# nickirk/pymes

Hardware: AMD Instinct MI355X
Metric: ccsd_iteration_time (lower is better)
Workload: dtype f64

## Files before the change

include/pymes_amd.h:

```cpp
#ifndef PYMES_AMD_H
#define PYMES_AMD_H

#include <stdint.h>

#ifdef __cplusplus
extern "C" {
#endif

typedef struct pymes_ctx pymes_ctx;

const char* pymes_last_error(void);
const char* pymes_backend(void);
int pymes_ctx_create(pymes_ctx** out, int device, int no, int nv, uint64_t workspace_bytes );
int pymes_ctx_destroy(pymes_ctx* ctx);
int pymes_ctx_set_stream(pymes_ctx* ctx, void* hip_stream);
int pymes_ctx_sync(pymes_ctx* ctx);
int pymes_ctx_workspace(pymes_ctx* ctx, uint64_t* capacity_bytes, uint64_t* high_water_bytes);

int pymes_malloc(pymes_ctx* ctx, uint64_t bytes, void** dev_ptr);
int pymes_free(pymes_ctx* ctx, void* dev_ptr);
int pymes_live_allocations(int64_t* n);
int pymes_mem_info(pymes_ctx* ctx, uint64_t* free_bytes, uint64_t* total_bytes);
int pymes_dress_generation(pymes_ctx* ctx, uint64_t* n);

// ... 154 lines not shown
                      double* e_out_host);
int pymes_ccd_energy(pymes_ctx* ctx, const double* t2_dev, double* e_out_host);

int pymes_ueg_eval_2b(pymes_ctx* ctx, int n_p, int n_ele, int imax, int mode, double L, double k_cutoff, double gamma,
                      int lattice_cutoff, const int32_t* k_int_host, const int32_t* index_map_host, double* V_dev);

int pymes_ueg_eval_2b_corr(pymes_ctx* ctx, int n_p, int n_ele, int imax, int mode, double L, int lattice_cutoff,
                           int correlator, const double* params_host, const int32_t* k_int_host,
                           const int32_t* index_map_host, double* V_dev);
int pymes_ueg_eval_2b_tab(pymes_ctx* ctx, int n_p, int n_ele, int imax, int mode, double L, int lattice_cutoff,
                          const int32_t* k_int_host, const int32_t* index_map_host, const double* tab_scalar_host,
                          const double* tab_array_host, int64_t tab_len, double* V_dev);

int pymes_dots(pymes_ctx* ctx, int npairs, const double* const* x_dev, const double* const* y_dev, int64_t n,
               double* out_host);
int pymes_dots_var(pymes_ctx* ctx, int npairs, const double* const* x_dev, const double* const* y_dev,
                   const int64_t* n, double* out_host);
int pymes_lincomb(pymes_ctx* ctx, double* out_dev, int nx, const double* const* x_dev, const double* c_host,
                  int64_t n);
int pymes_gemm_group_begin(pymes_ctx* ctx);
int pymes_gemm_group_end(pymes_ctx* ctx, int64_t* launches, int64_t* products);
int pymes_gram(pymes_ctx* ctx, int m, int n, const double* const* x_dev, const double* const* y_dev, int64_t len,
               double* out_host);
int pymes_lincomb_multi(pymes_ctx* ctx, int m, int n, const double* const* x_dev, const double* c_host,
                        const double* beta_host, double* const* y_dev, int64_t len);
int pymes_diis_mix(pymes_ctx* ctx, double* state_host, int ntypes, int m, int was_full, const double* const* err_hist_dev,
                   const double* const* err_new_dev, const int64_t* sizes, const double* const* amp_hist_dev,
                   double* const* out_dev);
int pymes_diis_step(pymes_ctx* ctx, double* state_dev, int npairs, const double* const* x_dev, const double* const* y_dev,
                    const int64_t* n, int ntypes, int m, int was_full);
int pymes_diis_solve(double* state_host, const double* overlaps_host, int ntypes, int m, int was_full);
int pymes_lincomb_dev(pymes_ctx* ctx, double* out_dev, int nx, const double* const* x_dev, const double* coeff_dev,
                      int64_t n);
int pymes_cmul(pymes_ctx* ctx, const double* mr_dev, const double* mi_dev, const double* xr_dev, const double* xi_dev,
               double* yr_dev, double* yi_dev, int64_t n);

int pymes_hf_fock_matrix(pymes_ctx* ctx, const double* h_host, double* f_host);

int pymes_fcidump_header(const char* path, int* n_elec, int* n_orb);
int pymes_fcidump_read_host(const char* path, int is_tc, double* e_core, double* eps_host, double* h_host,
                            double* V_host);
int pymes_fcidump_load(pymes_ctx* ctx, const char* path, int is_tc, double* e_core, double* eps_host, double* h_host,
                       int64_t* n_two_electron_lines);

int pymes_packed_header(const char* path, int* kind, int* n_elec, int* n_orb, int* naux);
int pymes_packed_load(pymes_ctx* ctx, const char* path, double* e_core, double* eps_host, double* h_host);
int pymes_packed_write(pymes_ctx* ctx, const char* path, int n_elec, double e_core, const double* eps_host,
                       const double* h_host);
int pymes_packed_write_factors(const char* path, int n_elec, int n_orb, int naux, double e_core, const double* eps_host,
                               const double* h_host, const double* B_host);

typedef struct pymes_eom pymes_eom;
int pymes_eom_sigma_prepare(pymes_ctx* ctx, const double* f_host, const double* t2_dev, int dressed, pymes_eom** out);
int pymes_eom_sigma_flags(pymes_eom* h, int* flags);
int pymes_eom_sigma_apply(pymes_eom* h, int k, const double* const* u1_dev, const double* const* u2_dev, const int* sym,
                          double* const* s1_dev, double* const* s2_dev);
int pymes_eom_diagonals(pymes_ctx* ctx, const double* f_host, const double* t2_dev, int dressed, double* d1_dev, double* d2_dev);
int pymes_scratch_trim(pymes_ctx* ctx);
int pymes_eom_sigma_destroy(pymes_eom* h);

#define PYMES_IPEA_IP 0
#define PYMES_IPEA_EA 1
typedef struct pymes_ipea pymes_ipea;
int pymes_ipea_sigma_prepare(pymes_ctx* ctx, const double* f_host, const double* t2_dev, int dressed, int kind, pymes_ipea** out);
int pymes_ipea_sigma_flags(pymes_ipea* h, int* flags);
int pymes_ipea_sigma_apply(pymes_ipea* h, int k, const double* const* r1_dev, const double* const* r2_dev, double* const* s1_dev,
// ... 44 lines not shown
```

pymes_amd/_lib.py:

```python
import ctypes as C
import os

import numpy as np

_HERE = os.path.dirname(os.path.abspath(__file__))
DEFAULT_PATH = os.environ.get("PYMES_AMD_LIBRARY") or os.path.join(_HERE, "lib", "libpymes_amd.so")

c_double_p = C.POINTER(C.c_double)
c_i64_p = C.POINTER(C.c_int64)


class ShardBuffers(C.Structure):
    _fields_ = [(k, C.c_void_p) for k in ("ETd", "ETx", "L", "QK", "Tall", "W", "Xvv", "P", "R1", "S")]

c_pp = C.POINTER(C.c_void_p)

SIGNATURES = {
    "pymes_last_error": (C.c_char_p, []),
    "pymes_backend": (C.c_char_p, []),
    "pymes_ctx_create": (C.c_int, [c_pp, C.c_int, C.c_int, C.c_int, C.c_uint64]),
    "pymes_ctx_destroy": (C.c_int, [C.c_void_p]),
    "pymes_ctx_set_stream": (C.c_int, [C.c_void_p, C.c_void_p]),
    "pymes_ctx_sync": (C.c_int, [C.c_void_p]),
    "pymes_ctx_workspace": (C.c_int, [C.c_void_p, C.POINTER(C.c_uint64), C.POINTER(C.c_uint64)]),
# ... 125 lines not shown
    "pymes_ccsd_sharded_finish": (C.c_int, [C.c_void_p] * 6 + [C.POINTER(C.c_int)]),
    "pymes_ccsd_sharded_energy": (C.c_int, [C.c_void_p, C.c_int, C.c_void_p]),
    "pymes_ccsd_sharded_await": (C.c_int, [C.c_void_p, C.c_void_p, C.c_void_p]),
    "pymes_cshift_inv": (C.c_int, [C.c_void_p, C.c_void_p] + [C.c_double] * 5 + [C.c_void_p, C.c_void_p, C.c_int64]),
    "pymes_eom_sigma_prepare": (C.c_int, [C.c_void_p, C.c_void_p, C.c_void_p, C.c_int, C.c_void_p]),
    "pymes_eom_sigma_flags": (C.c_int, [C.c_void_p, C.c_void_p]),
    "pymes_eom_sigma_apply": (C.c_int, [C.c_void_p, C.c_int] + [C.c_void_p] * 5),
    "pymes_eom_diagonals": (C.c_int, [C.c_void_p, C.c_void_p, C.c_void_p, C.c_int, C.c_void_p, C.c_void_p]),
    "pymes_scratch_trim": (C.c_int, [C.c_void_p]),
    "pymes_eom_sigma_destroy": (C.c_int, [C.c_void_p]),
    "pymes_eom_sigma_apply_left": (C.c_int, [C.c_void_p, C.c_int] + [C.c_void_p] * 5),
    "pymes_lambda_step": (C.c_int, [C.c_void_p] * 5 + [C.c_double, C.c_double, C.c_int, C.c_int] + [C.c_void_p] * 5),
    "pymes_rdm1": (C.c_int, [C.c_void_p] * 5 + [C.c_double, C.c_void_p]),
    "pymes_ipea_sigma_prepare": (C.c_int, [C.c_void_p, C.c_void_p, C.c_void_p, C.c_int, C.c_int, C.c_void_p]),
    "pymes_ipea_sigma_flags": (C.c_int, [C.c_void_p, C.c_void_p]),
    "pymes_ipea_sigma_apply": (C.c_int, [C.c_void_p, C.c_int] + [C.c_void_p] * 4),
    "pymes_ipea_sigma_apply_left": (C.c_int, [C.c_void_p, C.c_int] + [C.c_void_p] * 4),
    "pymes_ipea_dyson": (C.c_int, [C.c_void_p] * 4 + [C.c_int] + [C.c_void_p] * 6),
    "pymes_ipea_sigma_diagonals": (C.c_int, [C.c_void_p, C.c_void_p, C.c_void_p]),
    "pymes_ipea_sigma_correction": (C.c_int, [C.c_void_p, C.c_int, C.c_void_p, C.c_void_p, C.c_void_p, C.c_void_p, C.c_double,
                                              C.c_void_p, C.c_int64, C.c_int64, C.c_void_p]),
    "pymes_ipea_sigma_destroy": (C.c_int, [C.c_void_p]),
    "pymes_tdm1": (C.c_int, [C.c_void_p] * 5 + [C.c_int] + [C.c_void_p] * 7),
    "pymes_eom_correction": (C.c_int, [C.c_void_p, C.c_int, C.c_void_p, C.c_void_p, C.c_void_p, C.c_void_p, C.c_double,
                                       C.c_void_p, C.c_int64, C.c_int64, C.c_void_p]),
    "pymes_diis_mix": (C.c_int, [C.c_void_p, C.c_void_p, C.c_int, C.c_int, C.c_int, c_pp, c_pp, c_i64_p, c_pp, c_pp]),
    "pymes_diis_solve": (C.c_int, [C.c_void_p, C.c_void_p, C.c_int, C.c_int, C.c_int]),
    "pymes_diis_step": (C.c_int, [C.c_void_p, C.c_void_p, C.c_int, c_pp, c_pp, c_i64_p, C.c_int, C.c_int, C.c_int]),
    "pymes_gemm_group_begin": (C.c_int, [C.c_void_p]),
    "pymes_gemm_group_end": (C.c_int, [C.c_void_p, c_i64_p, c_i64_p]),
    "pymes_gram": (C.c_int, [C.c_void_p, C.c_int, C.c_int, c_pp, c_pp, C.c_int64, c_double_p]),
    "pymes_lincomb_multi": (C.c_int, [C.c_void_p, C.c_int, C.c_int, c_pp, C.c_void_p, C.c_void_p, c_pp, C.c_int64]),
    "pymes_lincomb_dev": (C.c_int, [C.c_void_p, C.c_void_p, C.c_int, c_pp, C.c_void_p, C.c_int64]),
    "pymes_stats": (C.c_int, [C.c_void_p, C.c_int, c_i64_p, c_double_p, c_i64_p, c_double_p]),
    "pymes_prof_enable": (C.c_int, [C.c_void_p, C.c_int]),
    "pymes_prof_reset": (C.c_int, [C.c_void_p]),
    "pymes_prof_query": (C.c_int, [C.c_void_p, C.c_int, c_i64_p, c_i64_p, c_double_p, c_double_p]),
}

PYMES_DCD, PYMES_USE_DRESSED, PYMES_SKIP_LADDER, PYMES_SYM_LADDER, PYMES_SYM_RINGS = 1, 2, 4, 8, 16
PYMES_OWNER_TILES = 1 << 21
PYMES_REUSE_LAYOUTS = 32
PYMES_T1_ZERO = 1 << 20
PYMES_SLAB_RINGS_ONLY, PYMES_SLAB_LADDERS_ONLY = 64, 128
PYMES_DRESS_ABIJ_REDUCED = 1 << 16


class PymesError(RuntimeError):
    pass


class Library:

    BACKEND = "hip-gfx950"

    def __init__(self, path=None):
        path = path or DEFAULT_PATH
        if not os.path.exists(path):
            raise PymesError(
                f"{path} not found: build the HIP extension first (python -c 'import __graft_entry__ as g; "
                "g.build()' or make -C pymes_amd/csrc).  pymes_amd has no CPU fallback.")
        self.path = path
        self.dll = C.CDLL(path)
        for name, (res, args) in SIGNATURES.items():
            fn = getattr(self.dll, name)
            fn.restype, fn.argtypes = res, args
        self.backend = self.dll.pymes_backend().decode()
        if self.backend != self.BACKEND:
            raise PymesError(f"{path} reports backend '{self.backend}', expected '{self.BACKEND}'")

    def call(self, name, *args):
        rc = getattr(self.dll, name)(*args)
        if rc != 0:
            raise PymesError(f"{name}: {self.dll.pymes_last_error().decode()}")


# ... 22 lines not shown
```

pymes_amd/csrc/capi.cpp:

```cpp
#include <chrono>
#include <cstdio>
#include <cstring>
#include <exception>
#include <algorithm>
#include <mutex>
#include <set>
#include <string>
#include <vector>

#include "../../include/pymes_amd.h"
#include "diis_small.h"
#include "engine.h"
#include "eom.h"
#include "fcidump.h"
#include "packed.h"

using pymes::Engine;
using pymes::TView;

struct pymes_ctx {
    Engine* e;
};
struct pymes_eom {
    pymes::EomSigma* s;
// ... 338 lines not shown
}
int pymes_shard_rows_ptr(pymes_ctx* ctx, const double** vp, const double** vm, int64_t* row0, int64_t* row1, int64_t* ldp,
                         int64_t* ldm) {
    return guarded([&] {
        need(vp, "vp"); need(vm, "vm"); need(row0, "row0"); need(row1, "row1"); need(ldp, "ldp"); need(ldm, "ldm");
        E(ctx).shard_rows(vp, vm, row0, row1, ldp, ldm);
    });
}
int pymes_set_orbital_energies(pymes_ctx* ctx, const double* eo, const double* ev) {
    return guarded([&] {
        need(eo, "eps_o");
        need(ev, "eps_v");
        E(ctx).set_orbital_energies(eo, ev);
    });
}

int pymes_mp2(pymes_ctx* ctx, double shift, double* t2, double* e_out) {
    return guarded([&] {
        need(t2, "t2");
        need(e_out, "e_out");
        E(ctx).mp2(shift, t2, e_out);
    });
}
int pymes_ccsd_dress_fock(pymes_ctx* ctx, const double* f, const double* t1, double* fd) {
    return guarded([&] {
        need(f, "f"); need(t1, "t1"); need(fd, "fd");
        E(ctx).dress_fock(f, t1, fd);
    });
}
int pymes_ccsd_residuals(pymes_ctx* ctx, const double* f, const double* t1, const double* t2, uint32_t flags, double* r1,
                         double* r2) {
    return guarded([&] {
        need(f, "f"); need(t1, "t1"); need(t2, "t2"); need(r1, "r1"); need(r2, "r2");
        if (flags & ~(PYMES_DCD | PYMES_T1_ZERO)) throw pymes::Error("ccsd_residuals: flags are PYMES_DCD | PYMES_T1_ZERO");
        E(ctx).ccsd_residuals(f, t1, t2, (flags & PYMES_DCD) | ((flags & PYMES_T1_ZERO) ? Engine::kT1Zero : 0u), r1, r2);
    });
}
int pymes_ccsd_iterate(pymes_ctx* ctx, const double* f, double* t1, double* t2, uint32_t flags, double level_shift, double delta,
                       double* dt1, double* dt2, double* out6) {
    return guarded([&] {
        need(f, "f"); need(t1, "t1"); need(t2, "t2"); need(dt1, "dt1"); need(dt2, "dt2"); need(out6, "out");
        if (flags & ~(PYMES_DCD | PYMES_T1_ZERO)) throw pymes::Error("ccsd_iterate: flags are PYMES_DCD | PYMES_T1_ZERO");
        Engine& e = E(ctx);
        if (e.capturing()) throw pymes::Error("ccsd_iterate reads the energy back: not inside a launch graph");
        e.ccsd_iterate(f, t1, t2, (flags & PYMES_DCD) | ((flags & PYMES_T1_ZERO) ? Engine::kT1Zero : 0u), level_shift, delta, dt1,
                       dt2, out6);
    });
}
int pymes_ccsd_release(pymes_ctx* ctx) {
    return guarded([&] {
        Engine& e = E(ctx);
        if (e.capturing()) throw pymes::Error("ccsd_release while a launch graph is being recorded");
        e.release_residual_buffers();
    });
}
int pymes_ccsd_dress_V(pymes_ctx* ctx, const double* t1, uint32_t mask) {
    return guarded([&] {
        need(t1, "t1");
        E(ctx).dress_V(t1, mask);
    });
}
int pymes_ccsd_dress_V_slab(pymes_ctx* ctx, const double* t1, uint32_t mask, int p_begin, int p_end, int q_begin,
                            int q_end) {
    return guarded([&] {
        need(t1, "t1");
        const int64_t cut[4] = {p_begin, p_end, q_begin, q_end};
        E(ctx).dress_V(t1, mask, cut);
    });
// ... 187 lines not shown
}
int pymes_ccsd_dress_abcd_rows(pymes_ctx* ctx, const double* t1, int a0, int a1, int lower_only) {
    return guarded([&] {
        need(t1, "t1");
        E(ctx).dress_abcd_rows(t1, a0, a1, lower_only != 0);
    });
}
int pymes_cc_update(pymes_ctx* ctx, double* t, double* dt, const double* r, double shift, double delta, int rank) {
    return guarded([&] {
        need(t, "t"); need(dt, "dt"); need(r, "r");
        E(ctx).cc_update(t, dt, r, shift, delta, rank);
    });
}
int pymes_cc_update_to(pymes_ctx* ctx, double* t_out, double* dt, const double* t_in, const double* r, double shift,
                       double delta, int rank) {
    return guarded([&] {
        need(t_out, "t_out"); need(dt, "dt"); need(t_in, "t_in"); need(r, "r");
        E(ctx).cc_update_to(t_out, dt, t_in, r, shift, delta, rank);
    });
}
int pymes_energy_norms(pymes_ctx* ctx, const double* f, const double* t1, const double* t2, const double* dt2,
                       double* out) {
    return guarded([&] {
        need(t2, "t2"); need(out, "out");
        if ((f == nullptr) != (t1 == nullptr)) throw pymes::Error("f and t1 must be given together");
        E(ctx).energy_norms(f, t1, t2, dt2, out);
    });
}
int pymes_energy_norms_start(pymes_ctx* ctx, const double* f, const double* t1, const double* t2, const double* dt2, int* slot) {
    return guarded([&] {
        need(t2, "t2"); need(slot, "slot");
        if ((f == nullptr) != (t1 == nullptr)) throw pymes::Error("f and t1 must be given together");
        *slot = E(ctx).energy_norms_start(f, t1, t2, dt2);
    });
}
int pymes_energy_norms_wait(pymes_ctx* ctx, int slot, double* out) {
    return guarded([&] {
        need(out, "out");
        Eq(ctx).energy_norms_wait(slot, out);
    });
}
int pymes_readback_start(pymes_ctx* ctx, const double* dev_ptr, int n, int* slot) {
    return guarded([&] {
        need(dev_ptr, "dev_ptr"); need(slot, "slot");
        *slot = dev::readback_start(dev_ptr, n, E(ctx).stream);
    });
}
int pymes_readback_wait(pymes_ctx* ctx, int slot, double* out, int n) {
    return guarded([&] {
        need(out, "out");
        Eq(ctx);
        dev::readback_wait(slot, out, n);
    });
}
int pymes_energy_norms_pairs(pymes_ctx* ctx, const double* f, const double* t1, const double* tc, const double* dtc,
                             int rank, int world, double* out) {
    return guarded([&] {
        need(tc, "tc"); need(out, "out");
        if ((f == nullptr) != (t1 == nullptr)) throw pymes::Error("f and t1 must be given together");
        E(ctx).energy_norms_pairs(f, t1, tc, dtc, rank, world, out);
    });
}
int pymes_set_collectives(pymes_ctx* ctx, const pymes_collectives* table) {
    return guarded([&] {
        if (!table) {
            E(ctx).set_collectives(nullptr);
// ... 137 lines not shown
        need(params, "params");
        if (mode == 0) throw pymes::Error("ueg: mode 0 (Coulomb) has no correlator");
        if (correlator < 1 || correlator > 6) throw pymes::Error("ueg: correlator must be 1..6 (0 = trunc: pymes_ueg_eval_2b)");
        ueg_eval(ctx, n_p, n_ele, imax, mode, L, 0.0, 1.0, lattice_cutoff, k_int, index_map, nullptr, nullptr, 0, V, correlator, params);
    });
}
int pymes_ueg_eval_2b_tab(pymes_ctx* ctx, int n_p, int n_ele, int imax, int mode, double L, int lattice_cutoff,
                          const int32_t* k_int, const int32_t* index_map, const double* tab_scalar, const double* tab_array,
                          int64_t tab_len, double* V) {
    return guarded([&] {
        need(tab_scalar, "tab_scalar"); need(tab_array, "tab_array");
        if (mode == 0) throw pymes::Error("ueg: mode 0 (Coulomb) has no correlator");
        ueg_eval(ctx, n_p, n_ele, imax, mode, L, 0.0, 1.0, lattice_cutoff, k_int, index_map, tab_scalar, tab_array, tab_len, V);
    });
}

int pymes_dots(pymes_ctx* ctx, int npairs, const double* const* x, const double* const* y, int64_t n,
               double* out) {
    return guarded([&] {
        need(x, "x"); need(y, "y"); need(out, "out");
        if (npairs < 0 || npairs > 16) throw pymes::Error("dots: 0..16 pairs");
        int64_t len[16];
        for (int i = 0; i < npairs; ++i) len[i] = n;
        dev::dots(npairs, x, y, len, out, E(ctx).stream);
    });
}
int pymes_dots_var(pymes_ctx* ctx, int npairs, const double* const* x, const double* const* y, const int64_t* n,
                   double* out) {
    return guarded([&] {
        need(x, "x"); need(y, "y"); need(n, "n"); need(out, "out");
        dev::dots(npairs, x, y, n, out, E(ctx).stream);
    });
}
int pymes_lincomb(pymes_ctx* ctx, double* out, int nx, const double* const* x, const double* c, int64_t n) {
    return guarded([&] {
        need(out, "out"); need(x, "x"); need(c, "c");
        dev::lincomb(out, nx, x, c, n, E(ctx).stream);
    });
}

int pymes_gemm_group_begin(pymes_ctx* ctx) {
    return guarded([&] { dev::gemm_group_begin(Eq(ctx).stream); });
}
int pymes_gemm_group_end(pymes_ctx* ctx, int64_t* launches, int64_t* products) {
    return guarded([&] {
        Eq(ctx);
        dev::gemm_group_end();
        long l = 0, p = 0;
        dev::gemm_group_stats(&l, &p);
        if (launches) *launches = l;
        if (products) *products = p;
    });
}
int pymes_gram(pymes_ctx* ctx, int m, int n, const double* const* x, const double* const* y, int64_t len, double* out) {
    return guarded([&] {
        need(x, "x"); need(y, "y"); need(out, "out");
        if (m < 0 || n < 0 || len < 0) throw pymes::Error("gram: negative size");
        for (int i = 0; i < m; ++i) need(x[i], "x[i]");
        for (int j = 0; j < n; ++j) need(y[j], "y[j]");
        dev::gram(m, n, x, y, len, out, E(ctx).stream);
    });
}
int pymes_lincomb_multi(pymes_ctx* ctx, int m, int n, const double* const* x, const double* c, const double* beta,
                        double* const* y, int64_t len) {
    return guarded([&] {
        need(y, "y");
        if (m < 0 || n < 0 || len < 0) throw pymes::Error("lincomb_multi: negative size");
        if (m > 0) { need(x, "x"); need(c, "c"); }
        for (int i = 0; i < m; ++i) need(x[i], "x[i]");
        for (int j = 0; j < n; ++j) need(y[j], "y[j]");
        dev::lincomb_multi(m, n, x, c, beta, y, len, E(ctx).stream);
    });
}

int pymes_diis_step(pymes_ctx* ctx, double* state, int npairs, const double* const* x, const double* const* y, const int64_t* n,
                    int ntypes, int m, int was_full) {
    return guarded([&] {
        need(state, "state"); need(x, "x"); need(y, "y"); need(n, "n");
        dev::diis_step(state, npairs, x, y, n, ntypes, m, was_full, E(ctx).stream);
    });
}
int pymes_diis_solve(double* state_host, const double* overlaps_host, int ntypes, int m, int was_full) {
    return guarded([&] {
        need(state_host, "state"); need(overlaps_host, "overlaps");
        if (ntypes < 1 || m < 1 || m > 8) throw pymes::Error("diis_solve: need ntypes >= 1, 1 <= m <= 8");
        diis_small::step(state_host, overlaps_host, ntypes, m, was_full);
    });
}
int pymes_diis_mix(pymes_ctx* ctx, double* state_host, int ntypes, int m, int was_full, const double* const* err_hist,
                   const double* const* err_new, const int64_t* sizes, const double* const* amp_hist, double* const* out) {
    return guarded([&] {
        need(state_host, "state"); need(err_hist, "err_hist"); need(err_new, "err_new"); need(sizes, "sizes");
        need(amp_hist, "amp_hist"); need(out, "out");
        if (ntypes < 1 || m < 1 || m > 8 || ntypes * m > 16) throw pymes::Error("diis_mix: need ntypes * m <= 16, m <= 8");
        Engine& e = E(ctx);
        const double* x[16];
        const double* y[16];
        int64_t n[16];
        for (int t = 0; t < ntypes; ++t)
            for (int i = 0; i < m; ++i) {
                x[t * m + i] = err_hist[t * m + i];
                y[t * m + i] = err_new[t];
                n[t * m + i] = sizes[t];
            }
        double ov[16];
        dev::dots(ntypes * m, x, y, n, ov, e.stream);
        diis_small::step(state_host, ov, ntypes, m, was_full);
        if (state_host[91] == 2.0)
            throw pymes::Error("DIIS: the subspace matrix is singular or not finite (numpy.linalg.LinAlgError in pymes/mixer/diis.py:85-95)");
        for (int t = 0; t < ntypes; ++t) dev::lincomb(out[t], m, amp_hist + t * m, state_host + 82, sizes[t], e.stream);
    });
}
int pymes_lincomb_dev(pymes_ctx* ctx, double* out, int nx, const double* const* x, const double* coeff_dev, int64_t n) {
    return guarded([&] {
        need(out, "out"); need(x, "x"); need(coeff_dev, "coeff");
        dev::lincomb_dev(out, nx, x, coeff_dev, n, E(ctx).stream);
    });
}
int pymes_cmul(pymes_ctx* ctx, const double* mr, const double* mi, const double* xr, const double* xi, double* yr, double* yi,
               int64_t n) {
    return guarded([&] {
        need(mr, "mr"); need(mi, "mi"); need(xr, "xr"); need(xi, "xi"); need(yr, "yr"); need(yi, "yi");
        dev::cmul(mr, mi, xr, xi, yr, yi, n, E(ctx).stream);
    });
}

int pymes_cshift_inv(pymes_ctx* ctx, const double* d, double zr, double zi, double hr, double hi, double shift, double* mr,
                     double* mi, int64_t n) {
    return guarded([&] {
        need(d, "d"); need(mr, "mr"); need(mi, "mi");
        dev::cshift_inv(d, zr, zi, hr, hi, shift, mr, mi, n, E(ctx).stream);
    });
}

int pymes_eom_sigma_prepare(pymes_ctx* ctx, const double* f_host, const double* t2, int dressed, pymes_eom** out) {
    return guarded([&] {
        need(out, "out");
        *out = nullptr;
        need(f_host, "f_host"); need(t2, "t2");
        Engine& e = E(ctx);
        e.refuse_if_sharded("EOM sigma");
        if (e.capturing()) throw pymes::Error("eom_sigma_prepare while a launch graph is being recorded");
        pymes::EomSigma* s = new pymes::EomSigma(e, f_host, t2, dressed != 0);
// ... 383 lines not shown
```

pymes_amd/csrc/cc.cpp:

```cpp
#include <algorithm>
#include <cstdio>
#include <cstring>
#include <cstdlib>
#include <vector>

#include "../../include/pymes_amd.h"
#include "engine.h"

#include <cmath>

namespace pymes {
static_assert(Engine::kT1Zero == PYMES_T1_ZERO && Engine::kOwnerTiles == PYMES_OWNER_TILES,
              "the engine's flag bits are the public ones");

namespace {
inline int64_t lpitch(int64_t n) { return (n + 15) & ~int64_t(15); }
inline TView packed_rows(double* p, int64_t rows, int64_t cols) { return slice(make_view(p, {rows, lpitch(cols)}), 1, 0, cols); }
constexpr int P_klij = 0, P_ijka = 1, P_ijak = 2, P_ijab = 3, P_iajk = 4, P_iajb = 5, P_iabj = 6, P_iabc = 7,
              P_aibc = 11, P_abij = 12, P_abic = 13, P_abci = 14, P_abcd = 15;
}

double* Engine::get_static(const std::string& key) {
    auto it = static_.find(key);
    if (it != static_.end()) return it->second;
// ... 130 lines not shown
            ArenaScope s2(arena);
            TView Z = ov2(), Q = ov2();
            contract(1.0, Td, "dkai", Vx, "cldk", 0.0, Z, "aicl");
            permute(-1.0, T, "cblj", 0.0, Q, "clbj");
            permute(1.0, T, "bclj", 1.0, Q, "clbj");
            contract(1.0, Z, "aicl", Q, "clbj", 1.0, Exd, "aibj");
        }
        Rx = ov2();
        TView X1 = ov2();
        contract(1.0, Tx, "ajdk", Vx, "cldk", 0.0, X1, "ajcl");
        contract(1.0, X1, "ajcl", Tx, "clbi", 0.0, Rx, "ajbi");
    }

    permute(1.0, Rd, "aibj", 1.0, R, "abij");
    if (quad) permute(1.0, Rx, "ajbi", 1.0, R, "abij");
    permute(1.0, Exd, "aibj", 1.0, R, "abij");
    permute(1.0, Exd, "bjai", 1.0, R, "abij");
    permute(1.0, Exx, "ajbi", 1.0, R, "abij");
    permute(1.0, Exx, "biaj", 1.0, R, "abij");
    permute(1.0, Exn, "abij", 1.0, R, "abij");
    permute(1.0, Exn, "baji", 1.0, R, "abij");
}

void Engine::ensure_xs() {
    if (!xs_oo_) xs_oo_ = static_cast<double*>(dev::dmalloc(sizeof(double) * no * no));
    if (!xs_vv_) xs_vv_ = static_cast<double*>(dev::dmalloc(sizeof(double) * nv * nv));
}

bool Engine::ring_fold_enabled() {
    if (const char* e = getenv("PYMES_RING_FOLD")) return atoi(e) != 0;
    return true;
}

void Engine::pair_layouts_of(const double* t2, bool want_td) {
    const int64_t o = no, v = nv, ov = o * v;
    for (int i = want_td ? 0 : 1; i < 3; ++i)
        if (!lay_[i]) {
            if (capturing_) throw Error("pair_layouts_of: the pair layouts must exist before a launch graph is recorded (run one eager pass first)");
            lay_[i] = static_cast<double*>(dev::dmalloc(sizeof(double) * ov * ov));
        }
    lay_t2_ = nullptr;
    if (dev::fused_pair_kernels_ok(no)) {
        dev::t2_layouts(t2, want_td ? lay_[0] : nullptr, lay_[1], lay_[2], no, nv, stream);
        stats.permute_calls++;
        stats.permute_bytes += 8.0 * (want_td ? 5.0 : 4.0) * double(ov * ov);
    } else {
        TView T = make_view(const_cast<double*>(t2), {v, v, o, o});
        TView t4 = make_view(lay_[0], {v, o, v, o});
        if (want_td) permute(1.0, T, "abij", 0.0, t4, "aibj");
        t4.p = lay_[1];
        permute(1.0, T, "abij", 0.0, t4, "ajbi");
        t4.p = lay_[2];
        permute(2.0, T, "abij", 0.0, t4, "aibj");
        permute(-1.0, T, "baij", 1.0, t4, "aibj");
    }
    lay_t2_ = t2;
}

void Engine::residual_slab(const double* f, const double* t2, double* ETd_p, double* ETx_p, double* L, int rank,
                           int world, unsigned flags, const double* t1, double* QK, const double* P) {
    const bool dcd = flags & PYMES_DCD, dressed = flags & PYMES_USE_DRESSED,
               skip_ladder = flags & (PYMES_SKIP_LADDER | PYMES_SLAB_RINGS_ONLY), skip_rings = flags & PYMES_SLAB_LADDERS_ONLY;
    const bool quad = !dcd;
    const int64_t o = no, v = nv, nn = n, ov = o * v;
    if (world < 1 || rank < 0 || rank >= world) throw Error("residual_slab: bad rank/world");
    if (L && !skip_ladder) check_shard_rank("residual_slab", rank, world);
    const double w = quad ? 1.0 : 0.5;
    TView F = make_view(const_cast<double*>(f), {nn, nn});
    auto chunk = [&](int64_t rows, int64_t& lo, int64_t& hi) {
        const int64_t c = (rows + world - 1) / world;
        lo = std::min<int64_t>(rank * c, rows);
        hi = std::min<int64_t>(lo + c, rows);
    };
    if (L && !skip_ladder) {
        int64_t r0, r1;
        chunk(v * (v + 1) / 2, r0, r1);
        if (t1) {
            if (!QK) throw Error("residual_slab: QK buffer missing");
            int64_t q0, q1;
            chunk(o * v, q0, q1);
            ladder_t1(t1, t2, L, r0, r1, QK, q0, q1, dcd, P ? P + o * o : nullptr);
        } else {
            ladder_sym(t2, L, r0, r1, dressed, quad ? 1 : 2);
        }
    }
    if (skip_rings) return;
    ring_fold_.clear();
    int64_t c0, c1;
    chunk(ov, c0, c1);
    const int64_t nc = c1 - c0;
    if (nc <= 0) return;
    TView Viajb = block(P_iajb, dressed), Viabj = block(P_iabj, dressed);

    ArenaScope scope(arena);
    auto pairm = [&](double* p) { return make_view(p, {ov, ov}); };
    auto slab = [&]() { return make_view(arena.alloc(ov * nc), {ov, nc}); };
    const bool traces = !P && nc == ov;
    const bool fold = traces && ring_fold_enabled();
    pair_layouts_of(t2, !fold);
    TView Td = pairm(lay_[0]), Tx = pairm(lay_[1]), Ttd = pairm(lay_[2]);
    TView ETd = slice(pairm(ETd_p), 0, c0, c1), ETx = slice(pairm(ETx_p), 0, c0, c1);
    auto cols = [&](const TView& m) { return slice(m, 1, c0, c1); };
    const int64_t b0 = c0 / o, b1 = (c1 + o - 1) / o;
    auto load_cols = [&](double alpha, const TView& blk, const char* spec, const TView& dst) {
        TView src = slice(blk, 1, b0, b1);
        if (b0 * o == c0 && b1 * o == c1) {
            permute(alpha, src, spec, 0.0, make_view(dst.p, {v, o, b1 - b0, o}), "ckbj");
        } else {
            ArenaScope s2(arena);
            TView tmp = make_view(arena.alloc(ov * (b1 - b0) * o), {ov, (b1 - b0) * o});
            permute(alpha, src, spec, 0.0, make_view(tmp.p, {v, o, b1 - b0, o}), "ckbj");
            copy(slice(tmp, 1, c0 - b0 * o, c1 - b0 * o), dst);
        }
    };
    const bool row_form = nc != ov;
    if (row_form) {
        auto slabT = [&]() { return make_view(arena.alloc(nc * ov), {nc, ov}); };
        TView MT = slabT(), N1T = slabT();
        auto load_rows = [&](double alpha, const TView& blk, const char* spec, const TView& dst) {
            TView src = slice(blk, 1, b0, b1);
            if (b0 * o == c0 && b1 * o == c1) {
                permute(alpha, src, spec, 0.0, make_view(dst.p, {b1 - b0, o, v, o}), "bjck");
            } else {
                ArenaScope s2(arena);
                TView tmp = make_view(arena.alloc((b1 - b0) * o * ov), {(b1 - b0) * o, ov});
                permute(alpha, src, spec, 0.0, make_view(tmp.p, {b1 - b0, o, v, o}), "bjck");
                copy(slice(tmp, 0, c0 - b0 * o, c1 - b0 * o), dst);
            }
        };
        load_rows(2.0, Viabj, "kbcj", MT);
        load_rows(-1.0, Viajb, "kbjc", N1T);
        axpby(1.0, N1T, 1.0, MT);
// ... 1120 lines not shown
        contract(-1.0, t, "ak", S2, "ki", 1.0, R, "ai");
    }
    contract(-1.0, Tq, "ajbk", slice(block(P_ijka), 0, j0, j1), "jkib", 1.0, R, "ai");
    if (!have_vv) {
        TView S4 = make_view(arena.alloc(v * v), {v, v});
        contract(1.0, Tq, "ajbk", slice(block(P_ijab), 0, j0, j1), "jkcb", 0.0, S4, "ac");
        contract(-1.0, S4, "ac", t, "ci", 1.0, R, "ai");
    }
}

void Engine::cc_update(double* t, double* dt, const double* r, double shift, double delta, int rank) {
    if (rank != 2 && rank != 4) throw Error("cc_update: rank must be 2 (T1) or 4 (T2)");
    need_eps("cc_update");
    dev::cc_update(t, dt, r, eps_o, eps_v, shift, delta, no, nv, rank, stream);
}

void Engine::ccsd_residuals(const double* f, const double* t1, const double* t2, unsigned flags, double* r1, double* r2) {
    refuse_if_sharded("ccsd_residuals (single rank)");
    const int64_t o = no, v = nv, ov = o * v, npp = v * (v + 1) / 2;
    if (!res_ETd_) {
        if (capturing_) throw Error("ccsd_residuals: the staging buffers must exist before a launch graph is recorded (run one eager pass first)");
        double* got[5] = {nullptr, nullptr, nullptr, nullptr, nullptr};
        const int64_t want[5] = {(o + v) * (o + v), ov * ov, ov * ov, npp * o * o, ov * o * o};
        try {
            for (int i = 0; i < 5; ++i) got[i] = scratch_get(want[i]);
        } catch (...) {
            for (double* p : got)
                if (p) scratch_put(p);
            throw;
        }
        res_fd_ = got[0]; res_ETd_ = got[1]; res_ETx_ = got[2]; res_L_ = got[3]; res_QK_ = got[4];
    }
    const unsigned dcd = flags & PYMES_DCD;
    const unsigned sym = PYMES_SYM_LADDER | PYMES_SYM_RINGS;
    if (flags & PYMES_T1_ZERO) {
        residual_slab(f, t2, res_ETd_, res_ETx_, res_L_, 0, 1, dcd | sym);
        singles_residual_partial(f, t1, t2, r1, 0, 1, true);
        residual_finish(f, t2, res_ETd_, res_ETx_, res_L_, r2, dcd | sym | PYMES_REUSE_LAYOUTS);
        return;
    }
    dress_fock(f, t1, res_fd_);
    dress_V(t1, (1u << pattern_of_name("klij")) | (1u << pattern_of_name("iajb")) | (1u << pattern_of_name("iabj")));
    residual_slab(res_fd_, t2, res_ETd_, res_ETx_, res_L_, 0, 1, dcd | sym | PYMES_USE_DRESSED, t1, res_QK_);
    singles_residual_partial(res_fd_, t1, t2, r1, 0, 1, true);
    residual_finish(res_fd_, t2, res_ETd_, res_ETx_, res_L_, r2, dcd | sym | PYMES_USE_DRESSED | PYMES_REUSE_LAYOUTS, t1, res_QK_);
}

void Engine::ccsd_iterate(const double* f, double* t1, double* t2, unsigned flags, double shift, double delta, double* dt1,
                          double* dt2, double out[6]) {
    refuse_if_sharded("ccsd_iterate (single rank)");
    const int64_t o = no, v = nv;
    if (!res_r1_) {
        if (capturing_) throw Error("ccsd_iterate: the staging buffers must exist before a launch graph is recorded");
        double* r1 = scratch_get(v * o);
        try {
            res_r2_ = scratch_get(v * v * o * o);
        } catch (...) {
            scratch_put(r1);
            throw;
        }
        res_r1_ = r1;
    }
    ccsd_residuals(f, t1, t2, flags, res_r1_, res_r2_);
    cc_update_to(t1, dt1, t1, res_r1_, shift, delta, 2);
    cc_update_to(t2, dt2, t2, res_r2_, shift, delta, 4);
    energy_norms(f, t1, t2, dt2, out);
}

void Engine::set_collectives(const Collectives* c) {
    if (t2_in_flight_) {
        t2_in_flight_ = false;
        dev::phase_sync();
        if (coll_.wait(coll_.user, t2_ticket_, stream) != 0) throw Error("collective hook: wait failed");
    }
    if (!c) {
        coll_ = Collectives();
        coll_set_ = false;
        return;
    }
    if (!c->allreduce_start || !c->allgather_start || !c->wait) throw Error("set_collectives: allreduce_start, allgather_start and wait are required");
    if (c->world < 1 || c->rank < 0 || c->rank >= c->world) throw Error("set_collectives: need 0 <= rank < world");
    coll_ = *c;
    coll_set_ = true;
}

namespace {
struct Hooks {
    const Engine::Collectives& c;
    void* stream;
    int64_t allreduce(double* buf, int64_t n) const {
        dev::gemm_group_sync();
        dev::phase_sync();
        int64_t t = 0;
        if (c.allreduce_start(c.user, buf, n, stream, &t) != 0) throw Error("collective hook: allreduce_start failed");
        return t;
    }
    int64_t allgather(double* buf, int64_t chunk) const {
        dev::gemm_group_sync();
        dev::phase_sync();
// ... 206 lines not shown
                                stream);
    h.wait(h.allreduce(b.S, 6));
    const int slot = dev::readback_start(b.S, 6, stream);
    t2_ticket_ = h.allgather(b.Tall, c * 2 * o2);
    t2_in_flight_ = true;
    h.mark("energy + norms (pairs)");
    return slot;
}

void Engine::ccsd_sharded_energy(int slot, double out[6]) {
    double r[6];
    dev::readback_wait(slot, r, 6);
    out[0] = 2.0 * r[0];
    out[1] = 2.0 * r[1];
    out[2] = -1.0 * r[2];
    out[3] = r[3];
    out[4] = r[4];
    out[5] = r[5];
}

void Engine::release_residual_buffers() {
    if (!graphs_.empty()) {
        release_wanted_ = true;
        return;
    }
    release_wanted_ = false;
    for (double** p : {&res_fd_, &res_ETd_, &res_ETx_, &res_L_, &res_QK_, &res_r1_, &res_r2_}) {
        if (*p) scratch_put(*p);
        *p = nullptr;
    }
}

void Engine::cc_update_to(double* t_out, double* dt, const double* t_in, const double* r, double shift, double delta,
                          int rank) {
    if (rank != 2 && rank != 4) throw Error("cc_update: rank must be 2 (T1) or 4 (T2)");
    need_eps("cc_update");
    dev::cc_update_to(t_out, dt, t_in, r, eps_o, eps_v, shift, delta, no, nv, rank, stream);
}

int Engine::energy_norms_start(const double* f, const double* t1, const double* t2, const double* dt2) {
    return dev::energy_norms_start(f, t1, t2, get_static("Edir"), get_static("Eex"), dt2, no, nv, stream);
}
void Engine::energy_norms_wait(int slot, double out[6]) {
    double r[6];
    dev::readback_wait(slot, r, 6);
    out[0] = 2.0 * r[0];
    out[1] = 2.0 * r[1];
    out[2] = -1.0 * r[2];
    out[3] = r[3];
    out[4] = r[4];
    out[5] = r[5];
}

void Engine::energy_norms(const double* f, const double* t1, const double* t2, const double* dt2, double out[6]) {
    double r[6];
    dev::energy_norms(f, t1, t2, get_static("Edir"), get_static("Eex"), dt2, no, nv, r, stream);
    out[0] = 2.0 * r[0];
    out[1] = 2.0 * r[1];
    out[2] = -1.0 * r[2];
    out[3] = r[3];
    out[4] = r[4];
    out[5] = r[5];
}

void Engine::energy_norms_pairs(const double* f, const double* t1, const double* tc, const double* dtc, int rank, int world,
                                double out[6]) {
    int64_t r0, r1;
    pair_chunk(rank, world, r0, r1);
    double r[6];
    dev::energy_norms_pairs(f, t1, tc, get_static("Edir"), get_static("Eex"), dtc, no, nv, r0, r1, rank == 0, r, stream);
    out[0] = 2.0 * r[0];
    out[1] = 2.0 * r[1];
    out[2] = -1.0 * r[2];
    out[3] = r[3];
    out[4] = r[4];
    out[5] = r[5];
}

void Engine::ccsd_energy(const double* f, const double* t1, const double* t2, double out[3]) {
    double r[6];
    energy_norms(f, t1, t2, nullptr, r);
    out[0] = r[0];
    out[1] = r[1];
    out[2] = r[2];
}

void Engine::ccd_energy(const double* t2, double out[2]) {
// ... 426 lines not shown
```

pymes_amd/csrc/device_api.h:

```cpp
#pragma once
#include <cstddef>
#include <cstdint>

namespace dev {

typedef void* stream_t;

const char* backend_name();
void  set_device(int ordinal);
void* dmalloc(size_t bytes);
void* try_dmalloc(size_t bytes);
void  dfree(void* p);
void  memcpy_h2d(void* d, const void* h, size_t bytes, stream_t s);
void  memcpy_d2h(void* h, const void* d, size_t bytes, stream_t s);
void  memcpy_d2d(void* d, const void* s_, size_t bytes, stream_t s);
void  memset_zero(void* d, size_t bytes, stream_t s);
void  stream_sync(stream_t s);
size_t mem_free_bytes();
size_t mem_total_bytes();
stream_t stream_create();
void  stream_destroy(stream_t s);
int64_t live_allocations();
typedef void* event_t;
event_t event_create();
// ... 48 lines not shown
void phase_stats(long* tasks, long* launches, long* levels, long* flushes);

struct Permute {
    int rank;
    int64_t dim[6];
    int64_t s_in[6], s_out[6];
    double alpha, beta;
    const double* in; double* out;
};
void permute(const Permute& p, stream_t s);

void mp2_amplitudes(double* t, const double* w, const double* eo, const double* ev, double shift,
                    int no, int nv, stream_t s);
void cc_update(double* t, double* dt, const double* r, const double* eo, const double* ev, double shift,
               double delta, int no, int nv, int rank, stream_t s);
void dots(int npairs, const double* const* x, const double* const* y, const int64_t* n, double* out_host,
          stream_t s);
void energy_norms(const double* f, const double* t1, const double* t2, const double* Edir, const double* Eex,
                  const double* dt2, int no, int nv, double out_host[6], stream_t s);
int energy_norms_start(const double* f, const double* t1, const double* t2, const double* Edir, const double* Eex,
                       const double* dt2, int no, int nv, stream_t s);
int readback_start(const double* dev_ptr, int n, stream_t s);
void readback_wait(int slot, double* out_host, int n);
void energy_norms_pairs(const double* f, const double* t1, const double* tc, const double* Edir, const double* Eex,
                        const double* dtc, int no, int nv, int64_t r0, int64_t r1, bool with_t1, double out_host[6],
                        stream_t s);
void energy_norms_pairs_dev(const double* f, const double* t1, const double* tc, const double* Edir, const double* Eex,
                            const double* dtc, int no, int nv, int64_t r0, int64_t r1, bool with_t1, double* out_dev,
                            stream_t s);
void exchange_asymmetry(const double* A, const double* B, const int64_t d[4], double out_host[2], stream_t s);
void cc_update_to(double* t_out, double* dt, const double* t_in, const double* r, const double* eo, const double* ev,
                  double shift, double delta, int no, int nv, int rank, stream_t s);
void lincomb(double* out, int nx, const double* const* x, const double* c, int64_t n, stream_t s);
void gram(int m, int n, const double* const* x, const double* const* y, int64_t len, double* out_host, stream_t s);
void lincomb_multi(int m, int n, const double* const* x, const double* c, const double* beta, double* const* y, int64_t len,
                   stream_t s);
void diis_step(double* state, int npairs, const double* const* x, const double* const* y, const int64_t* n, int ntypes, int m,
               int was_full, stream_t s);
void lincomb_dev(double* out, int nx, const double* const* x, const double* coeff_dev, int64_t n, stream_t s);
void cmul(const double* mr, const double* mi, const double* xr, const double* xi, double* yr, double* yi, int64_t n, stream_t s);
void exchange_split(const double* u, double* us, double* w, double* dg, int no, int nv, stream_t s);
void sgn_ij_add(double* D, const double* R, int no, int nv, stream_t s);
void cshift_inv(const double* d, double zr, double zi, double hr, double hi, double shift, double* mr, double* mi, int64_t n,
                stream_t s);
int64_t eom_diag_ws_doubles(int no, int nv);
void eom_diagonals(const double* V, const double* T, const double* dai, const double* iaai, const double* iaia, const double* ijij,
                   const double* abab, double* d1, double* d2, int no, int nv, double* ws, stream_t s);
void tau_build(double* tau, const double* t2, const double* t1, int no, int nv, stream_t s);

void ladder_pack_V(const double* V, double* Vp, double* Vm, int nr, int nc, int64_t rp0, int64_t rp1, stream_t s,
                   int64_t ldvp = 0, int64_t ldvm = 0);
void ladder_pack_V_factors(const double* B, double* Vp, double* Vm, int naux, int n, int no, int64_t rp0, int64_t rp1,
                           stream_t s, int64_t ldvp, int64_t ldvm);
int64_t triples_partial_doubles(int nv, int64_t nt);
void triples_energy(const double* W, int64_t nt, int64_t t0, const double* Vijab, const double* t1, const double* eps,
                    double* partial, double* out, int no, int nv, stream_t s);
int64_t fno_density_partial_doubles(int noa, int nv);
void fno_density(const double* Vijab, const double* eps_o, const double* eps_v, int no, int nf, int nv, double* partial,
                 double* D, double* e, stream_t s);
bool ladder_dress_ok(int no, int nv);
int64_t ladder_dress_ws_doubles(int no, int nv);
void ladder_dress(const double* V, const double* Pk, const double* t1, double* W, int no, int nv, int64_t ld, int64_t row0,
                  int64_t row1, double sgn, double* ws, stream_t s);
enum { PACK_ROW_HALF = 1, PACK_AM_PROWS = 2, PACK_COL_HALF = 4, PACK_AM_PCOLS = 8 };
void ladder_pack_T(const double* X, const double* t1, double* Sp, double* Am, int nc, int nr, int flags, int64_t ldp,
                   int64_t ldm, stream_t s, int64_t rp0 = 0, int64_t rp1 = -1);
// ... 88 lines not shown
```

pymes_amd/csrc/engine.cpp:

```cpp
#include "engine.h"

#include <algorithm>
#include <cstdio>
#include <cstdlib>
#include <cstring>
#include <tuple>

namespace pymes {

TView make_view(double* p, int rank, const int64_t* dims, const int64_t* strides) {
    if (rank < 0 || rank > 6) throw Error("tensor rank must be 0..6");
    TView t;
    t.p = p;
    t.rank = rank;
    int64_t s = 1;
    for (int i = rank - 1; i >= 0; --i) {
        t.dim[i] = dims[i];
        t.st[i] = strides ? strides[i] : s;
        s *= dims[i];
    }
    return t;
}
TView make_view(double* p, std::initializer_list<int64_t> dims) {
    int64_t d[6];
// ... 731 lines not shown
                                     double*, double*, stream_t) {
    throw std::runtime_error("ipea_pack: not available in this backend");
}
__attribute__((weak)) void ipea_assemble(int, const double*, const double*, const double*, const double*, int, int, int,
                                         double* const*, double* const*, stream_t) {
    throw std::runtime_error("ipea_assemble: not available in this backend");
}
__attribute__((weak)) void ipea_unpack(int, const double*, const double*, const double*, const double*, const double*, int, int, int,
                                       double* const*, double* const*, stream_t) {
    throw std::runtime_error("ipea_unpack: not available in this backend");
}
__attribute__((weak)) void ipea_dyson_assemble(const DysonParts&, int, int, int, int, stream_t) {
    throw std::runtime_error("ipea_dyson_assemble: not available in this backend");
}
__attribute__((weak)) void ipea_diagonals(const double*, const double*, int, int, int, double*, double*, stream_t) {
    throw std::runtime_error("ipea_diagonals: not available in this backend");
}
__attribute__((weak)) int64_t ipea_correction_ws_doubles(int, int64_t) { return 1; }
__attribute__((weak)) void ipea_correction(int, const double* const*, const double* const*, const double*, const double*, double,
                                           double* const*, int64_t, int64_t, int64_t, double*, double*, stream_t) {
    throw std::runtime_error("ipea_correction: not available in this backend");
}
__attribute__((weak)) int64_t lambda_assemble_ws_doubles(int) { return 1; }
__attribute__((weak)) void lambda_assemble(const LambdaParts&, int, int, stream_t) {
    throw std::runtime_error("lambda_assemble: not available in this backend");
}
__attribute__((weak)) void rdm1_assemble(const double*, const double*, const double*, const double*, const double*, int, int,
                                         double, double*, stream_t) {
    throw std::runtime_error("rdm1_assemble: not available in this backend");
}
__attribute__((weak)) void tdm1_assemble(const Tdm1Parts&, int, int, int, stream_t) {
    throw std::runtime_error("tdm1_assemble: not available in this backend");
}
}
```

pymes_amd/csrc/engine.h:

```cpp
#pragma once
#include <cstdint>
#include <map>
#include <set>
#include <stdexcept>
#include <string>
#include <vector>

#include "device_api.h"

namespace pymes {

struct TView {
    double* p = nullptr;
    int rank = 0;
    int64_t dim[6] = {1, 1, 1, 1, 1, 1};
    int64_t st[6] = {0, 0, 0, 0, 0, 0};
    int64_t size() const {
        int64_t n = 1;
        for (int i = 0; i < rank; ++i) n *= dim[i];
        return n;
    }
};

TView make_view(double* p, std::initializer_list<int64_t> dims);
// ... 106 lines not shown
    void singles_residual(const double* fd, const double* t1, const double* t2, double* r1);
    void singles_residual_partial(const double* fd, const double* t1, const double* t2, double* r1, int rank, int world,
                                  bool reuse_layouts = false);
    void doubles_residual(const double* f, const double* t2, double* r2, unsigned flags);
    void ladder(const double* t2, double* r2, int a0, int a1, bool dressed, double beta);
    void ladder_sym(const double* t2, double* L, int64_t row0, int64_t row1, bool dressed, int hole = 0);
    void ladder_sym_multi(const double* const* xs, int k, double* L_all, bool dressed);
    void ladder_sym_adjoint(const double* x, double* LS, double* LA, bool dressed);
    void ladder_sym_adjoint_multi(const double* const* xs, int k, double* LS, double* LA, bool dressed);
    int64_t ladder_adjoint_pitch(bool symmetric_half) const {
        const int64_t o = no, opp = o * (o + 1) / 2, opm = o * (o - 1) / 2;
        return ((symmetric_half ? opp : opm) + 2) & ~int64_t(1);
    }
    void hole_ladder_packed_multi(const double* const* xs, const double* const* Is, const double* const* ys, int k, double* L_all);
    void hole_ladder_packed(const double* x, const double* I, double* L, int64_t row0, int64_t row1,
                            const double* y = nullptr);
    void ladder_sym_unpack(const double* L, double* r2, double beta);
    void residual_slab(const double* f, const double* t2, double* ETd, double* ETx, double* L, int rank, int world,
                       unsigned flags, const double* t1 = nullptr, double* QK = nullptr, const double* P = nullptr);
    int64_t slab_prepare_ws_doubles() const;
    void slab_prepare(const double* t2, double* P, int rank, int world, unsigned flags);
    void residual_finish(const double* f, const double* t2, const double* ETd, const double* ETx, const double* L,
                         double* r2, unsigned flags, const double* t1 = nullptr, const double* QK = nullptr);
    void residual_finish_pairs(const double* f, const double* t2, const double* ETd, const double* ETx, const double* L,
                               double* Rc, unsigned flags, const double* t1, const double* QK, int rank, int world,
                               const double* Xvv_in = nullptr);
    void pair_chunk(int rank, int world, int64_t& r0, int64_t& r1) const;
    void amplitude_side_abij(const double* t1, const double* QK, const TView& N, int64_t a0, int64_t a1, int64_t b1,
                             bool with_partner, double beta = 1.0);
    void ladder_t1(const double* t1, const double* t2, double* L, int64_t row0, int64_t row1, double* QK, int64_t q0,
                   int64_t q1, bool dcd, const double* J = nullptr);
    void dress_abcd_rows(const double* t1, int a0, int a1, bool lower_only);
    static constexpr unsigned kT1Zero = 1u << 20;
    void ccsd_residuals(const double* f, const double* t1, const double* t2, unsigned flags, double* r1, double* r2);
    void ccsd_iterate(const double* f, double* t1, double* t2, unsigned flags, double shift, double delta, double* dt1,
                      double* dt2, double out[6]);
    void release_residual_buffers();
    void cc_update(double* t, double* dt, const double* r, double shift, double delta, int rank);
    void cc_update_to(double* t_out, double* dt, const double* t_in, const double* r, double shift, double delta, int rank);
    void ccsd_energy(const double* f, const double* t1, const double* t2, double out[3]);
    void ccd_energy(const double* t2, double out[2]);
    void energy_norms(const double* f, const double* t1, const double* t2, const double* dt2, double out[6]);
    int energy_norms_start(const double* f, const double* t1, const double* t2, const double* dt2);
    void energy_norms_wait(int slot, double out[6]);
    void energy_norms_pairs(const double* f, const double* t1, const double* tc, const double* dtc, int rank, int world,
                            double out[6]);
    struct Collectives {
        void* user = nullptr;
        int rank = 0, world = 1;
        int (*allreduce_start)(void* user, double* buf, int64_t n, void* stream, int64_t* ticket) = nullptr;
        int (*allgather_start)(void* user, double* buf, int64_t chunk, void* stream, int64_t* ticket) = nullptr;
        int (*wait)(void* user, int64_t ticket, void* stream) = nullptr;
        void (*mark)(void* user, const char* phase) = nullptr;
    };
    struct ShardBuffers {
        double *ETd, *ETx, *L, *QK, *Tall, *W, *Xvv, *P, *R1, *S;
    };
    void set_collectives(const Collectives* c);
    bool has_collectives() const { return coll_set_; }
    typedef int (*alltoallv_fn)(void* user, const double* send, const int64_t* send_counts, double* recv,
                                const int64_t* recv_counts, void* stream, int64_t* ticket);
    void set_alltoallv(alltoallv_fn fn) { alltoallv_ = fn; }
    void set_owner_tile_buffers(double* send, double* recv) { xs_ = send; xr_ = recv; }
    void owner_tile_sizes(int rank, int world, int64_t* send_doubles, int64_t* recv_doubles) const;
    static constexpr unsigned kOwnerTiles = 1u << 21;
    void ccsd_sharded_residuals(const double* f, double* fd, const double* t1, double* t2, const ShardBuffers& b,
                                unsigned flags, double* rc);
    void ccd_sharded_residuals(const double* f, double* t2, const ShardBuffers& b, unsigned flags, double* rc);
    int ccsd_sharded_finish(const double* f, const double* t1, const double* tc, const double* dtc, const ShardBuffers& b);
    void ccsd_sharded_energy(int slot, double out[6]);
    void ccsd_sharded_await(double* t2, const ShardBuffers& b);
    static int64_t triples_count(int no);
    double ccsd_t(const double* eps_host, const double* t1, const double* t2, int64_t t_begin, int64_t t_end, double* per_triple);
    void check_hermitian(const char* who, const char* why);
    double fno_density(const double* Vijab, int n_frozen, double* D_host);
    void derive_from(Engine& src, int n_frozen, const double* C_host, int nv_dst);
    void invalidate_static();

    double* eps_o = nullptr;
    double* eps_v = nullptr;
    bool eps_set = false;
    void need_eps(const char* who) const;
    double* splitk_ws() const { return splitk_ws_; }
    int64_t splitk_ws_doubles() const { return splitk_doubles_; }

  private:
    double* lay_[3] = {nullptr, nullptr, nullptr};
    const double* lay_t2_ = nullptr;
    void pair_layouts_of(const double* t2, bool want_td);
    struct FoldTag {
        const double* t2 = nullptr;
        const double* etd = nullptr;
        bool is(const double* t, const double* e) const { return t2 && t2 == t && etd == e; }
        void set(const double* t, const double* e) { t2 = t; etd = e; }
        void clear() { t2 = etd = nullptr; }
    } ring_fold_;
    static bool ring_fold_enabled();
    struct SumTag {
        const double* t2 = nullptr;
        int rank = 0, world = 0;
        bool is(const double* p, int r, int w) const { return t2 && t2 == p && rank == r && world == w; }
        void set(const double* p, int r, int w) { t2 = p; rank = r; world = w; }
        void clear() { t2 = nullptr; }
    };
    double ring_xd_ = 0.0;
    double* xs_oo_ = nullptr;
    double* xs_vv_ = nullptr;
    SumTag xs_oo_tag_, xs_vv_tag_;
    void ensure_xs();
    dev::stream_t own_stream_ = nullptr;
    std::set<void*> user_allocs_;
    Collectives coll_;
    alltoallv_fn alltoallv_ = nullptr;
    double *xs_ = nullptr, *xr_ = nullptr;
    struct Rect { int64_t r0, r1, c0, c1; };
    std::vector<Rect> owner_tile_rects(int from, int to, int world) const;
    int64_t owner_tiles_start(const ShardBuffers& b);
    void owner_tiles_finish(const ShardBuffers& b);
    bool coll_set_ = false, t2_in_flight_ = false;
    int64_t t2_ticket_ = 0;
    double *res_fd_ = nullptr, *res_ETd_ = nullptr, *res_ETx_ = nullptr, *res_L_ = nullptr, *res_QK_ = nullptr, *res_r1_ = nullptr,
           *res_r2_ = nullptr;
// ... 47 lines not shown
```

pymes_amd/csrc/kernels.hip:

```cpp
#include <hip/hip_runtime.h>
#include <type_traits>

#include <algorithm>
#include <atomic>
#include <chrono>
#include <cmath>
#include <cstdio>
#include <cstdlib>
#include <cstring>
#include <mutex>
#include <stdexcept>
#include <string>
#include <vector>

#include "device_api.h"
#include "diis_small.h"

#define HIP_CHECK(expr)                                                                   \
    do {                                                                                  \
        hipError_t err__ = (expr);                                                        \
        if (err__ != hipSuccess)                                                          \
            throw std::runtime_error(std::string("HIP error: ") + hipGetErrorString(err__) + \
                                     " at " __FILE__ ":" + std::to_string(__LINE__));     \
    } while (0)
// ... 2108 lines not shown
    const int p = no + 1;
    const long o2 = (long)no * no, ov = (long)no * nv, opp = (long)no * (no + 1) / 2;
    const long ab = ((long)a * nv + b) * o2, ba = ((long)b * nv + a) * o2;
    const long tab = (long)a * no * ov + (long)b * no, tba = (long)b * no * ov + (long)a * no;
    for (int e = threadIdx.x; e < o2; e += blockDim.x) {
        const int i = e / no, j = e - i * no;
        double v = N[ab + e] + D[tab + (long)i * ov + j] + X[tba + (long)i * ov + j];
        if (xd != 0.0) v += xd * X[tab + (long)i * ov + j];
        S[i * p + j] = v;
    }
    __syncthreads();
    for (int e = threadIdx.x; e < o2; e += blockDim.x) {
        const int j = e / no, i = e - j * no;
        double v = N[ba + e] + D[tba + (long)j * ov + i] + X[tab + (long)j * ov + i];
        if (xd != 0.0) v += xd * X[tba + (long)j * ov + i];
        S[i * p + j] += v;
    }
    __syncthreads();
    const double* __restrict__ row = L ? L + ((long)a * (a + 1) / 2 + b) * o2 : nullptr;
    for (int e = threadIdx.x; e < o2; e += blockDim.x) {
        const int i = e / no, j = e - i * no;
        const int ih = max(i, j), il = min(i, j);
        double ls = 0.0, la = 0.0;
        if (row) {
            ls = row[(long)ih * (ih + 1) / 2 + il];
            if (a != b && i != j) la = row[opp + (long)ih * (ih - 1) / 2 + il];
        }
        const double sgn = i > j ? 1.0 : -1.0;
        R[ab + e] = (V ? V[ab + e] : 0.0) + ls + sgn * la + S[i * p + j];
        if (a != b) R[ba + e] = (V ? V[ba + e] : 0.0) + ls - sgn * la + S[j * p + i];
    }
}
__global__ void __launch_bounds__(256) residual_assemble_kernel(const AssembleK k) { residual_assemble_body(k, blockIdx.x); }

__global__ void __launch_bounds__(256) energy_norms_pairs_kernel(const double* __restrict__ f, const double* __restrict__ t1,
                                                                 const double* __restrict__ tc, const double* __restrict__ Edir,
                                                                 const double* __restrict__ Eex, const double* __restrict__ dtc,
                                                                 int no, int nv, long r0, long npairs, int with_t1,
                                                                 double* __restrict__ partial) {
    __shared__ double sh[4];
    double s1 = 0.0, s2 = 0.0, s3 = 0.0, s4 = 0.0, s0 = 0.0, s5 = 0.0;
    const long o2 = (long)no * no;
    for (long tile = blockIdx.x; tile < 2 * npairs; tile += gridDim.x) {
        int a, b;
        unrank_pair(r0 + (tile >> 1), a, b);
        if (tile & 1) {
            if (a == b) continue;
            const int x = a; a = b; b = x;
        }
        const double* __restrict__ x = tc + tile * o2;
        const double* __restrict__ d = dtc ? dtc + tile * o2 : nullptr;
        const double* __restrict__ ed = Edir + ((long)a * nv + b) * o2;
        const double* __restrict__ ex = Eex + ((long)a * nv + b) * o2;
        for (int e = threadIdx.x; e < o2; e += blockDim.x) {
            const double v = x[e];
            double tau = v;
            if (t1) {
                const int i = e / no, j = e - i * no;
                tau += t1[a * no + i] * t1[b * no + j];
            }
            s1 += tau * ed[e];
            s2 += tau * ex[e];
            s3 += v * v;
            if (d) s4 += d[e] * d[e];
        }
    }
// ... 2033 lines not shown
        for (int i = 0; i < r; ++i) { k.dim[i] = m[i].n; k.s_in[i] = m[i].si; k.s_out[i] = m[i].so; }
        for (int i = r; i < 6; ++i) { k.dim[i] = 1; k.s_in[i] = 0; k.s_out[i] = 0; }
        if (phase) { record(PK_PERM_DIRECT, grid_for(total, 256, 256 * 32), 0, PermTaskK{k, total, 0, 0}); return; }
        launch_kernel(permute_direct_kernel, dim3(grid_for(total, 256, 256 * 32)), dim3(256), 0, st, k, total);
    }
}

void mp2_amplitudes(double* t, const double* w, const double* eo, const double* ev, double shift, int no, int nv,
                    stream_t s) {
    const long total = (long)nv * nv * no * no;
    if (!total) return;
    launch_kernel(mp2_amplitudes_kernel, dim3(grid_for(total)), dim3(256), 0, (hipStream_t)s, t, w, eo, ev,
                       shift, no, nv, total);
}

void cc_update_to(double* t_out, double* dt, const double* t_in, const double* r, const double* eo, const double* ev,
                  double shift, double delta, int no, int nv, int rank, stream_t s) {
    const long total = rank == 4 ? (long)nv * nv * no * no : (long)nv * no;
    if (!total) return;
    const CcUpdateK k{t_out, dt, t_in, r, eo, ev, shift, delta, no, nv, rank, total};
    const double cost = 32.0 * (double)total / 4.0e6;
    if (phase_open((hipStream_t)s) && phase_small(cost)) {
        PhaseRec& t = phase_push(PK_CC_UPDATE, 0, grid_for(total), 0, cost, k);
        phase_reads(t, {prange(t_in, total), prange(r, total), prange(eo, no), prange(ev, nv)});
        phase_writes(t, {prange(t_out, total), prange(dt, total)});
        return;
    }
    launch_kernel(cc_update_kernel, dim3(grid_for(total)), dim3(256), 0, (hipStream_t)s, k);
}
void cc_update(double* t, double* dt, const double* r, const double* eo, const double* ev, double shift,
               double delta, int no, int nv, int rank, stream_t s) {
    cc_update_to(t, dt, t, r, eo, ev, shift, delta, no, nv, rank, s);
}

static int launch_dots_stage1(int npairs, const double* const* x, const double* const* y, const int64_t* n, double* ws,
                              hipStream_t st) {
    DotPtrs p;
    long nmax = 0;
    bool vec = true;
    for (int i = 0; i < npairs; ++i) {
        p.x[i] = x[i]; p.y[i] = y[i]; p.n[i] = (long)n[i];
        nmax = std::max(nmax, p.n[i]);
        vec = vec && ((reinterpret_cast<uintptr_t>(x[i]) | reinterpret_cast<uintptr_t>(y[i])) & 15) == 0;
    }
    for (int i = npairs; i < 16; ++i) { p.x[i] = nullptr; p.y[i] = nullptr; p.n[i] = 0; }
    const long per = vec ? 512 : 256;
    const int nb = (int)std::max<long>(1, std::min<long>(kDotBlocks, (nmax + per - 1) / per));
    const DotsK k{p, ws, nb, npairs};
    double bytes = 0.0;
    for (int i = 0; i < npairs; ++i) bytes += 16.0 * (double)p.n[i];
    if (phase_open(st) && phase_small(bytes / 4.0e6)) {
        PhaseRec& t = phase_push(PK_DOTS1, vec ? 1 : 0, (long)nb * npairs, 0, bytes / 4.0e6, k);
        uintptr_t lo = ~(uintptr_t)0, hi = 0;
        for (int i = 0; i < npairs; ++i)
            for (const double* q : {p.x[i], p.y[i]}) {
                lo = std::min(lo, reinterpret_cast<uintptr_t>(q));
                hi = std::max(hi, reinterpret_cast<uintptr_t>(q) + 8 * (uintptr_t)p.n[i]);
            }
        phase_reads(t, {PhaseRange{lo, hi}});
        phase_writes(t, {prange(ws, 16L * kDotBlocks)});
        return nb;
    }
    if (vec) launch_kernel(dots_stage1_kernel<2>, dim3(nb * npairs), dim3(256), 0, st, k);
    else launch_kernel(dots_stage1_kernel<1>, dim3(nb * npairs), dim3(256), 0, st, k);
    return nb;
}
static void launch_dots_stage2(int npairs, double* ws, int nb, double* out_dev, hipStream_t st) {
    if (phase_open(st)) {
        PhaseRec& t = phase_push(PK_DOTS2, 0, npairs, 0, 1.0, Dots2K{ws, out_dev, nb});
        phase_reads(t, {prange(ws, 16L * kDotBlocks)});
        phase_writes(t, {prange(out_dev, npairs)});
        return;
    }
    launch_kernel(dots_stage2_kernel, dim3(npairs), dim3(256), 0, st, ws, nb, out_dev);
}

static void launch_dots_final(DotsFinalK k, double* ws, hipStream_t st) {
    {
        const int dv = current_device();
        std::lock_guard<std::mutex> lock(g_arrivals_mu);
        k.arrivals = g_arrivals[dv] + 32 * (g_arrivals_next[dv]++ % kArrivalSlots);
        k.pad_ = 0;
    }
    if (phase_open(st)) {
        PhaseRec& t = phase_push(PK_DOTS_FINAL, 0, k.npairs, 0, 1.0, k);
        phase_reads(t, {prange(ws, 16L * kDotBlocks)});
        return;
    }
    launch_kernel(dots_final_kernel, dim3(k.npairs), dim3(256), 0, st, k);
}

void dots(int npairs, const double* const* x, const double* const* y, const int64_t* n, double* out_host, stream_t s) {
    if (npairs <= 0) return;
    if (npairs > 16) throw std::runtime_error("dots: at most 16 pairs per call");
    hipStream_t st = (hipStream_t)s;
    const int dv = current_device();
    ensure_dot_ws(dv);
    const int nb = launch_dots_stage1(npairs, x, y, n, g_dot_ws[dv], st);
    void* hd = nullptr;
    HIP_CHECK(hipHostGetDevicePointer(&hd, g_dot_host[dv], 0));
    const long seq = ++g_dot_seq[dv];
    launch_dots_final(DotsFinalK{g_dot_ws[dv], static_cast<double*>(hd), reinterpret_cast<long*>(static_cast<double*>(hd) + 16), nullptr, 0u, seq, nb,
                                 npairs},
                      g_dot_ws[dv], st);
    phase_flush();
    if (!poll_flag(reinterpret_cast<const long*>(g_dot_host[dv] + 16), seq, st)) throw std::runtime_error("dots: the device never delivered the result");
    for (int i = 0; i < npairs; ++i) out_host[i] = g_dot_host[dv][i];
}

void diis_step(double* state, int npairs, const double* const* x, const double* const* y, const int64_t* n, int ntypes, int m,
               int was_full, stream_t s) {
    if (npairs != ntypes * m || npairs < 1 || npairs > 16 || m + 1 > diis_small::kMaxOrder)
        throw std::runtime_error("diis_step: bad sizes");
    hipStream_t st = (hipStream_t)s;
    const int dv = current_device();
    ensure_dot_ws(dv);
    const int nb = launch_dots_stage1(npairs, x, y, n, g_dot_ws[dv], st);
    double* out_dev = g_dot_ws[dv] + 16 * kDotBlocks;
    launch_dots_stage2(npairs, g_dot_ws[dv], nb, out_dev, st);
    launch_kernel(diis_step_kernel, dim3(1), dim3(64), 0, st, state, out_dev, ntypes, m, was_full);
}

void lincomb_dev(double* out, int nx, const double* const* x, const double* coeff_dev, int64_t n, stream_t s) {
    if (nx < 0 || nx > 8) throw std::runtime_error("lincomb_dev: at most 8 terms");
    if (n <= 0) return;
    LinPtrsDev p;
    for (int i = 0; i < 8; ++i) p.x[i] = i < nx ? x[i] : nullptr;
    launch_kernel(lincomb_dev_kernel, dim3(grid_for(n)), dim3(256), 0, (hipStream_t)s, out, p, coeff_dev, nx, (long)n);
}

int energy_norms_start(const double* f, const double* t1, const double* t2, const double* Edir, const double* Eex,
                       const double* dt2, int no, int nv, stream_t s) {
    gemm_group_flush();
    hipStream_t st = (hipStream_t)s;
    const int dv = current_device();
    ensure_dot_ws(dv);
    const long total = (long)nv * nv * no * no;
    const int nb = (int)std::max<long>(1, std::min<long>(kDotBlocks, (total + 255) / 256));
    const bool vec = (no % 2 == 0) && !((reinterpret_cast<uintptr_t>(t2) | reinterpret_cast<uintptr_t>(Edir) |
                                          reinterpret_cast<uintptr_t>(Eex) | reinterpret_cast<uintptr_t>(dt2)) & 15);
    const EnergyK k{f, t1, t2, Edir, Eex, dt2, g_dot_ws[dv], total, no, nv};
    const double cost = (dt2 ? 32.0 : 24.0) * (double)total / 4.0e6;
    if (phase_open(st) && phase_small(cost)) {
        PhaseRec& t = phase_push(PK_ENERGY, vec ? 1 : 0, nb, 0, cost, k);
        const long n = no + nv;
        phase_reads(t, {prange(t2, total), prange(Edir, total), prange(Eex, total), prange(dt2, dt2 ? total : 0),
                        prange(t1, t1 ? (long)no * nv : 0), prange(f, (t1 && f) ? n * n : 0)});
        phase_writes(t, {prange(g_dot_ws[dv], 16L * kDotBlocks)});
    } else {
        if (vec) launch_kernel(energy_norms_kernel<2>, dim3(nb), dim3(256), 0, st, k);
        else launch_kernel(energy_norms_kernel<1>, dim3(nb), dim3(256), 0, st, k);
    }
    double* out_pin = nullptr;
    long* flag = nullptr;
    long seq = 0;
    const int ticket = readback_reserve_flagged(dv, &out_pin, &flag, &seq);
    launch_dots_final(DotsFinalK{g_dot_ws[dv], out_pin, flag, nullptr, 0u, seq, nb, 6}, g_dot_ws[dv], st);
    phase_flush();
    return ticket;
}
void energy_norms(const double* f, const double* t1, const double* t2, const double* Edir, const double* Eex,
                  const double* dt2, int no, int nv, double out_host[6], stream_t s) {
    readback_wait_impl(energy_norms_start(f, t1, t2, Edir, Eex, dt2, no, nv, s), out_host, 6);
}
int readback_start(const double* dev_ptr, int n, stream_t s) {
    flush_deferred();
    return readback_start_impl(dev_ptr, n, (hipStream_t)s);
}
void readback_wait(int slot, double* out_host, int n) { readback_wait_impl(slot, out_host, n); }

void exchange_asymmetry(const double* A, const double* B, const int64_t d[4], double out_host[2], stream_t s) {
    hipStream_t st = (hipStream_t)s;
    const int dv = current_device();
    ensure_dot_ws(dv);
    const long total = (long)d[0] * d[1] * d[2] * d[3];
    out_host[0] = out_host[1] = 0.0;
    if (!total) return;
    unsigned long long* out_dev = reinterpret_cast<unsigned long long*>(g_dot_ws[dv] + 16 * kDotBlocks);
    HIP_CHECK(set_async(out_dev, 0, 2 * sizeof(unsigned long long), st));
    const long tr = (d[2] + 63) / 64, ts = (d[3] + 63) / 64, ntiles = d[0] * d[1] * tr * ts;
    const int self = (A == B && d[0] == d[1]) ? 1 : 0;
    const unsigned grid = (unsigned)std::min<long>(ntiles, 256L * 8);
    const bool vec = even(d[2]) && even(d[3]) && aligned16(A) && aligned16(B);
    if (vec)
        launch_kernel(exchange_asym_kernel<true>, dim3(grid), dim3(256), 0, st, A, B, (long)d[0], (long)d[1], (long)d[2],
                           (long)d[3], (int)tr, (int)ts, ntiles, self, out_dev);
    else
        launch_kernel(exchange_asym_kernel<false>, dim3(grid), dim3(256), 0, st, A, B, (long)d[0], (long)d[1], (long)d[2],
                           (long)d[3], (int)tr, (int)ts, ntiles, self, out_dev);
    HIP_CHECK(copy_async(g_dot_host[dv], out_dev, sizeof(double) * 2, hipMemcpyDeviceToHost, st));
    wait_idle(st);
    out_host[0] = g_dot_host[dv][0];
    out_host[1] = g_dot_host[dv][1];
}

void lincomb(double* out, int nx, const double* const* x, const double* c, int64_t n, stream_t s) {
    if (nx < 0 || nx > 8) throw std::runtime_error("lincomb: at most 8 terms");
    if (n <= 0) return;
    LinPtrs p;
    for (int i = 0; i < 8; ++i) { p.x[i] = i < nx ? x[i] : nullptr; p.c[i] = i < nx ? c[i] : 0.0; }
    const LinK k{out, p, (long)n, nx};
    const double cost = 8.0 * (double)(nx + 1) * (double)n / 4.0e6;
    if (phase_open((hipStream_t)s) && phase_small(cost)) {
        PhaseRec& t = phase_push(PK_LINCOMB, 0, grid_for(n), 0, cost, k);
        for (int i = 0; i < nx; ++i) phase_reads(t, {prange(x[i], n)});
        phase_writes(t, {prange(out, n)});
        return;
    }
    launch_kernel(lincomb_kernel, dim3(grid_for(n)), dim3(256), 0, (hipStream_t)s, k);
}

namespace {
template <int MM, int NN>
void gram_tile(const double* const* x, int mm, const double* const* y, int nn, long len, bool vec, int nblk, double* ws,
               double* tile_dev, hipStream_t st) {
    GramPtrs<MM, NN> p;
    for (int i = 0; i < MM; ++i) p.x[i] = x[i < mm ? i : 0];
    for (int j = 0; j < NN; ++j) p.y[j] = y[j < nn ? j : 0];
    if (vec) launch_kernel(gram_stage1_kernel<MM, NN, 2>, dim3(nblk), dim3(256), 0, st, p, len, ws);
    else launch_kernel(gram_stage1_kernel<MM, NN, 1>, dim3(nblk), dim3(256), 0, st, p, len, ws);
    launch_kernel(gram_stage2_kernel, dim3(MM * NN), dim3(256), 0, st, ws, nblk, MM * NN, tile_dev);
}
template <int MM>
void gram_tile_n(const double* const* x, int mm, const double* const* y, int nn, long len, bool vec, int nblk, double* ws,
                 double* tile_dev, hipStream_t st, int& NNout) {
    if (nn <= 1) { NNout = 1; gram_tile<MM, 1>(x, mm, y, nn, len, vec, nblk, ws, tile_dev, st); }
    else if (nn <= 2) { NNout = 2; gram_tile<MM, 2>(x, mm, y, nn, len, vec, nblk, ws, tile_dev, st); }
    else if (nn <= 3) { NNout = 3; gram_tile<MM, 3>(x, mm, y, nn, len, vec, nblk, ws, tile_dev, st); }
    else { NNout = 4; gram_tile<MM, 4>(x, mm, y, nn, len, vec, nblk, ws, tile_dev, st); }
}
template <int MM, int NN>
void lincomb_multi_tile(const double* const* x, int mm, const double* c, int ldc, const double* beta, double* const* y, int nn,
                        long len, bool vec, hipStream_t st) {
    LinMulti<MM, NN> p;
    for (int i = 0; i < MM; ++i) {
        p.x[i] = x[i < mm ? i : 0];
        for (int j = 0; j < NN; ++j) p.c[i][j] = (i < mm && j < nn) ? c[(long)i * ldc + j] : 0.0;
    }
    for (int j = 0; j < NN; ++j) { p.y[j] = y[j < nn ? j : 0]; p.beta[j] = j < nn ? beta[j] : 0.0; }
    const long nvec = vec ? len / 2 : len;
    const int nblk = (int)std::max<long>(1, std::min<long>(8192, (nvec + 255) / 256));
    if (vec) launch_kernel(lincomb_multi_kernel<MM, NN, 2>, dim3(nblk), dim3(256), 0, st, p, nn, len);
// ... 250 lines not shown

void ring_operands(const double* Viabj, const double* Viajb, double* M, double* N1, double a1, double a2, int no, int nv,
                   stream_t s) {
    if (no < 1 || nv < 1) return;
    const size_t lds = sizeof(double) * (size_t)no * 33;
    if (lds > 64 * 1024) throw std::runtime_error("ring_operands: nocc too large for the LDS tile");
    const RingOpK k{Viabj, Viajb, M, N1, a1, a2, no, nv};
    const long ov2 = (long)no * nv * no * nv;
    const double cost = 32.0 * (double)ov2 / 4.0e6;
    if (phase_open((hipStream_t)s) && phase_small(cost)) {
        PhaseRec& t = phase_push(PK_RING_OPERANDS, 0, (long)no * nv, (int)lds, cost, k);
        phase_reads(t, {prange(Viabj, ov2), prange(Viajb, ov2)});
        phase_writes(t, {prange(M, ov2), prange(N1, ov2)});
        return;
    }
    launch_kernel(ring_operands_kernel, dim3((unsigned)((long)no * nv)), dim3(256), lds, (hipStream_t)s, k);
}

void t2_layouts(const double* T, double* Td, double* Tx, double* Ttd, int no, int nv, stream_t s, double ca, double cb) {
    if (!fused_pair_kernels_ok(no)) throw std::runtime_error("t2_layouts: nocc too large for the LDS tile");
    const size_t lds = sizeof(double) * no * (no + 1);
    const LayoutsK k{T, Td, Tx, Ttd, ca, cb, no, nv};
    const bool res = ca == 2.0 && cb == -1.0;
    const long n4 = (long)nv * nv * no * no;
    const double cost = 40.0 * (double)n4 / 4.0e6;
    if (phase_open((hipStream_t)s) && phase_small(cost)) {
        PhaseRec& t = phase_push(PK_T2_LAYOUTS, res ? 1 : 0, (long)nv * nv, (int)lds, cost, k);
        phase_reads(t, {prange(T, n4)});
        phase_writes(t, {prange(Td, Td ? n4 : 0), prange(Tx, n4), prange(Ttd, n4)});
        return;
    }
    if (res) launch_kernel(t2_layouts_kernel<true>, dim3((unsigned)(nv * nv)), dim3(256), lds, (hipStream_t)s, k);
    else launch_kernel(t2_layouts_kernel<false>, dim3((unsigned)(nv * nv)), dim3(256), lds, (hipStream_t)s, k);
}

void residual_assemble(const double* V, const double* L, const double* N, const double* D, const double* X, double* R,
                       int no, int nv, stream_t s, double xd) {
    if (!fused_pair_kernels_ok(no)) throw std::runtime_error("residual_assemble: nocc too large for the LDS tile");
    const size_t lds = sizeof(double) * no * (no + 1);
    const AssembleK k{V, L, N, D, X, R, xd, no, nv};
    const long n4 = (long)nv * nv * no * no;
    const double cost = 48.0 * (double)n4 / 4.0e6;
    if (phase_open((hipStream_t)s) && phase_small(cost)) {
        PhaseRec& t = phase_push(PK_ASSEMBLE, 0, (long)nv * (nv + 1) / 2, (int)lds, cost, k);
        phase_reads(t, {prange(V, V ? n4 : 0), prange(L, L ? (long)nv * (nv + 1) / 2 * no * no : 0), prange(N, n4), prange(D, n4), prange(X, n4)});
        phase_writes(t, {prange(R, n4)});
        return;
    }
    launch_kernel(residual_assemble_kernel, dim3((unsigned)((long)nv * (nv + 1) / 2)), dim3(256), lds, (hipStream_t)s, k);
}

void scatter(double* dst, const int64_t* idx_host, const double* val_host, int64_t n, stream_t s) {
    if (n <= 0) return;
    long* idx = nullptr;
    double* val = nullptr;
    HIP_CHECK(hipMalloc(&idx, sizeof(long) * n));
    if (hipMalloc(&val, sizeof(double) * n) != hipSuccess) { (void)free_device(idx); throw std::runtime_error("scatter: out of device memory"); }
    hipStream_t st = (hipStream_t)s;
    HIP_CHECK(copy_async(idx, idx_host, sizeof(long) * n, hipMemcpyHostToDevice, st));
    HIP_CHECK(copy_async(val, val_host, sizeof(double) * n, hipMemcpyHostToDevice, st));
    const hipError_t e = try_launch_kernel(scatter_kernel, dim3(grid_for(n)), dim3(256), 0, st, dst, idx, val, (long)n);
    (void)sync_stream(st);
    (void)free_device(idx);
    (void)free_device(val);
    HIP_CHECK(e);
}
// ... 1240 lines not shown
```

pymes_amd/device.py:

```python
import ctypes as C
import weakref

import numpy as np

from . import _lib
from ._lib import PymesError, i64_array, ptr_array

BLOCK_NAMES = ("abci", "iabj", "iajk", "aijk", "klij", "aibj", "ijak", "abic",
               "iajb", "abcd", "iabc", "aijb", "ijka", "aibc", "ijab", "abij")


def pattern_of(name):
    return sum((1 << (3 - p)) for p, ch in enumerate(name) if ch in "abcd")


class DeviceArray:

    def __init__(self, ctx, ptr, shape, owned=True, keepalive=None):
        self.ctx, self.ptr, self.shape = ctx, int(ptr), tuple(int(s) for s in shape)
        self._owned, self._keep = owned, keepalive
        self.size = int(np.prod(self.shape)) if self.shape else 1

    @property
    def nbytes(self):
# ... 305 lines not shown
        return hold()

    def phase_stats(self):
        v = [C.c_int64() for _ in range(4)]
        self.lib.call("pymes_phase_stats", *[C.byref(x) for x in v])
        return dict(zip(("tasks", "launches", "levels", "flushes"), (int(x.value) for x in v)))

    @property
    def dress_generation(self):
        n = C.c_uint64()
        self.lib.call("pymes_dress_generation", self.handle, C.byref(n))
        return int(n.value)

    def mp2(self, t2, level_shift=0.0):
        e = (C.c_double * 2)()
        self.lib.call("pymes_mp2", self.handle, float(level_shift), C.c_void_p(t2.ptr), e)
        return e[0], e[1]

    def dress_fock(self, f, t1, out):
        self.lib.call("pymes_ccsd_dress_fock", self.handle, C.c_void_p(f.ptr), C.c_void_p(t1.ptr), C.c_void_p(out.ptr))
        return out

    def dress_V(self, t1, names, reduced_abij=False, q_range=None, p_range=None):
        mask = _lib.PYMES_DRESS_ABIJ_REDUCED if reduced_abij else 0
        for nm in names:
            mask |= 1 << pattern_of(nm)
        if q_range is not None or p_range is not None:
            p0, p1 = p_range if p_range is not None else (0, 0)
            q0, q1 = q_range if q_range is not None else (0, 0)
            self.lib.call("pymes_ccsd_dress_V_slab", self.handle, C.c_void_p(t1.ptr), mask, int(p0), int(p1), int(q0), int(q1))
        else:
            self.lib.call("pymes_ccsd_dress_V", self.handle, C.c_void_p(t1.ptr), mask)

    def ccsd_residuals(self, f, t1, t2, r1, r2, is_dcd=False, t1_zero=False):
        self.lib.call("pymes_ccsd_residuals", self.handle, C.c_void_p(f.ptr), C.c_void_p(t1.ptr), C.c_void_p(t2.ptr),
                      (_lib.PYMES_DCD if is_dcd else 0) | (_lib.PYMES_T1_ZERO if t1_zero else 0), C.c_void_p(r1.ptr),
                      C.c_void_p(r2.ptr))

    def ccsd_iterate(self, f, t1, t2, dt1, dt2, level_shift=0.0, delta=1.0, is_dcd=False, t1_zero=False):
        out = (C.c_double * 6)()
        self.lib.call("pymes_ccsd_iterate", self.handle, C.c_void_p(f.ptr), C.c_void_p(t1.ptr), C.c_void_p(t2.ptr),
                      (_lib.PYMES_DCD if is_dcd else 0) | (_lib.PYMES_T1_ZERO if t1_zero else 0), float(level_shift), float(delta),
                      C.c_void_p(dt1.ptr), C.c_void_p(dt2.ptr), out)
        return tuple(out)

    def ccsd_release(self):
        self.lib.call("pymes_ccsd_release", self.handle)

    def singles_residual(self, fd, t1, t2, out):
        self.lib.call("pymes_ccsd_singles_residual", self.handle, C.c_void_p(fd.ptr), C.c_void_p(t1.ptr),
                      C.c_void_p(t2.ptr), C.c_void_p(out.ptr))
        return out

    def singles_residual_partial(self, fd, t1, t2, out, rank, world, reuse_layouts=False):
        self.lib.call("pymes_ccsd_singles_residual_partial", self.handle, C.c_void_p(fd.ptr), C.c_void_p(t1.ptr),
                      C.c_void_p(t2.ptr), C.c_void_p(out.ptr), int(rank), int(world),
                      _lib.PYMES_REUSE_LAYOUTS if reuse_layouts else 0)
        return out

    def doubles_residual(self, f, t2, out, is_dcd=False, dressed=False, skip_ladder=False, sym_ladder=False,
                         sym_rings=None):
        sym_rings = sym_ladder if sym_rings is None else sym_rings
        flags = (_lib.PYMES_DCD if is_dcd else 0) | (_lib.PYMES_USE_DRESSED if dressed else 0) | \
                (_lib.PYMES_SKIP_LADDER if skip_ladder else 0) | (_lib.PYMES_SYM_LADDER if sym_ladder else 0) | \
                (_lib.PYMES_SYM_RINGS if sym_rings else 0)
        self.lib.call("pymes_doubles_residual", self.handle, C.c_void_p(f.ptr), C.c_void_p(t2.ptr),
                      C.c_void_p(out.ptr), flags)
        return out

    def ladder(self, t2, out, a_begin, a_end, dressed=False, beta=0.0):
        self.lib.call("pymes_ladder", self.handle, C.c_void_p(t2.ptr), C.c_void_p(out.ptr), int(a_begin), int(a_end),
                      int(dressed), float(beta))
        return out

    @staticmethod
    def _flags(is_dcd, dressed, skip_ladder=False, sym_ladder=False, sym_rings=False):
        return (_lib.PYMES_DCD if is_dcd else 0) | (_lib.PYMES_USE_DRESSED if dressed else 0) | \
               (_lib.PYMES_SKIP_LADDER if skip_ladder else 0) | (_lib.PYMES_SYM_LADDER if sym_ladder else 0) | \
               (_lib.PYMES_SYM_RINGS if sym_rings else 0)

    def residual_slab(self, f, t2, ETd, ETx, L, rank, world, is_dcd=False, dressed=False, t1=None, QK=None, P=None,
                      part=None):
        extra = {None: 0, "rings": _lib.PYMES_SLAB_RINGS_ONLY, "ladders": _lib.PYMES_SLAB_LADDERS_ONLY}[part]
        self.lib.call("pymes_residual_slab", self.handle, C.c_void_p(f.ptr), C.c_void_p(t2.ptr), C.c_void_p(ETd.ptr),
                      C.c_void_p(ETx.ptr), C.c_void_p(L.ptr if L is not None else 0), int(rank), int(world),
                      self._flags(is_dcd, dressed, False, True, True) | extra, C.c_void_p(t1.ptr if t1 is not None else 0),
                      C.c_void_p(QK.ptr if QK is not None else 0), C.c_void_p(P.ptr if P is not None else 0))

    def slab_prepare_ws(self):
        n = C.c_int64()
        self.lib.call("pymes_slab_prepare_ws", self.handle, C.byref(n))
        return n.value

    def slab_prepare(self, t2, P, rank, world, is_dcd=False):
        self.lib.call("pymes_slab_prepare", self.handle, C.c_void_p(t2.ptr), C.c_void_p(P.ptr), int(rank), int(world),
                      _lib.PYMES_DCD if is_dcd else 0)
        return P

# ... 39 lines not shown

    def pairs_supported(self):
        yes = C.c_int()
        self.lib.call("pymes_pairs_supported", self.handle, C.byref(yes))
        return bool(yes.value)

    def pairs_pack(self, full, xc, rank, world):
        self.lib.call("pymes_pairs_pack", self.handle, C.c_void_p(full.ptr), C.c_void_p(xc.ptr), int(rank), int(world))
        return xc

    def pairs_unpack(self, xc_all, full, world):
        self.lib.call("pymes_pairs_unpack", self.handle, C.c_void_p(xc_all.ptr), C.c_void_p(full.ptr), int(world))
        return full

    def dress_abcd_rows(self, t1, a_begin, a_end, lower_only=False):
        self.lib.call("pymes_ccsd_dress_abcd_rows", self.handle, C.c_void_p(t1.ptr), int(a_begin), int(a_end),
                      int(lower_only))

    def ladder_sym(self, t2, L, row_begin, row_end, dressed=False, hole_ladder=0):
        self.lib.call("pymes_ladder_sym", self.handle, C.c_void_p(t2.ptr), C.c_void_p(L.ptr), int(row_begin),
                      int(row_end), int(dressed), int(hole_ladder))
        return L

    def ladder_sym_multi(self, xs, L_all, dressed=False):
        self.lib.call("pymes_ladder_sym_multi", self.handle, ptr_array([x.ptr for x in xs]), len(xs), C.c_void_p(L_all.ptr),
                      int(dressed))
        return L_all

    def ladder_dress(self, V, Pk, t1, W, ld, r0, r1, minus_half=False):
        self.lib.call("pymes_ladder_dress", self.handle, C.c_void_p(V.ptr), C.c_void_p(Pk.ptr), C.c_void_p(t1.ptr),
                      C.c_void_p(W.ptr), int(ld), int(r0), int(r1), int(minus_half))
        return W

    def pair_layouts(self, x, Xx, Xt, Xd=None):
        self.lib.call("pymes_pair_layouts", self.handle, C.c_void_p(x.ptr), C.c_void_p(Xd.ptr if Xd is not None else 0),
                      C.c_void_p(Xx.ptr), C.c_void_p(Xt.ptr))

    def symmetrised_assemble(self, N, D, X, out, V=None, L=None):
        self.lib.call("pymes_symmetrised_assemble", self.handle, C.c_void_p(V.ptr if V is not None else 0),
                      C.c_void_p(L.ptr if L is not None else 0), C.c_void_p(N.ptr), C.c_void_p(D.ptr), C.c_void_p(X.ptr),
                      C.c_void_p(out.ptr))
        return out

    def hole_ladder_packed(self, x, I, L, row_begin, row_end, y=None):
        self.lib.call("pymes_hole_ladder_packed", self.handle, C.c_void_p(x.ptr), C.c_void_p(I.ptr), C.c_void_p(L.ptr),
                      int(row_begin), int(row_end), C.c_void_p(y.ptr if y is not None else 0))
        return L

    def hole_ladder_packed_multi(self, xs, Is, L_all, ys=None):
        k = len(xs)
        self.lib.call("pymes_hole_ladder_packed_multi", self.handle, ptr_array([x.ptr for x in xs]),
                      ptr_array([i.ptr for i in Is]), ptr_array([y.ptr for y in ys]) if ys is not None else None, k,
                      C.c_void_p(L_all.ptr))
        return L_all

    def ladder_sym_unpack(self, L, out, beta=1.0):
        self.lib.call("pymes_ladder_sym_unpack", self.handle, C.c_void_p(L.ptr), C.c_void_p(out.ptr), float(beta))
        return out

    def cc_update(self, t, dt, r, level_shift=0.0, delta=1.0):
        rank = len(t.shape)
        self.lib.call("pymes_cc_update", self.handle, C.c_void_p(t.ptr), C.c_void_p(dt.ptr), C.c_void_p(r.ptr),
                      float(level_shift), float(delta), rank)

    def cc_update_to(self, t_out, dt, t_in, r, level_shift=0.0, delta=1.0):
        self.lib.call("pymes_cc_update_to", self.handle, C.c_void_p(t_out.ptr), C.c_void_p(dt.ptr), C.c_void_p(t_in.ptr),
                      C.c_void_p(r.ptr), float(level_shift), float(delta), len(t_in.shape))

    def energy_norms(self, f, t1, t2, dt2=None):
        out = (C.c_double * 6)()
        self.lib.call("pymes_energy_norms", self.handle, C.c_void_p(f.ptr if f is not None else 0),
                      C.c_void_p(t1.ptr if t1 is not None else 0), C.c_void_p(t2.ptr),
                      C.c_void_p(dt2.ptr if dt2 is not None else 0), out)
        return tuple(out[:])

    def energy_norms_start(self, f, t1, t2, dt2=None):
        slot = C.c_int()
        self.lib.call("pymes_energy_norms_start", self.handle, C.c_void_p(f.ptr if f is not None else 0),
                      C.c_void_p(t1.ptr if t1 is not None else 0), C.c_void_p(t2.ptr),
                      C.c_void_p(dt2.ptr if dt2 is not None else 0), C.byref(slot))
        return slot.value

    def energy_norms_wait(self, slot):
        out = (C.c_double * 6)()
        self.lib.call("pymes_energy_norms_wait", self.handle, int(slot), out)
        return tuple(out[:])

    def readback_start(self, arr, n=None, offset=0):
        n = arr.size - offset if n is None else int(n)
        slot = C.c_int()
        self.lib.call("pymes_readback_start", self.handle, C.c_void_p(arr.ptr + 8 * int(offset)), n, C.byref(slot))
        return slot.value

    def readback_wait(self, slot, n):
        buf = (C.c_double * int(n))()
        self.lib.call("pymes_readback_wait", self.handle, int(slot), buf, int(n))
        return np.frombuffer(buf, dtype=np.float64).copy()

    def energy_norms_pairs(self, f, t1, tc, dtc, rank, world):
        out = (C.c_double * 6)()
        self.lib.call("pymes_energy_norms_pairs", self.handle, C.c_void_p(f.ptr if f is not None else 0),
                      C.c_void_p(t1.ptr if t1 is not None else 0), C.c_void_p(tc.ptr),
                      C.c_void_p(dtc.ptr if dtc is not None else 0), int(rank), int(world), out)
        return np.array(out[:])

    recording = False

    def graph_begin(self):
        self.lib.call("pymes_graph_begin", self.handle)
        self.recording = True

    def graph_end(self):
        g = C.c_void_p()
        self.recording = False
        self.lib.call("pymes_graph_end", self.handle, C.byref(g))
        return g

    def graph_abort(self):
        self.recording = False
        self.lib.call("pymes_graph_abort", self.handle)

    def graph_launch(self, g):
        self.lib.call("pymes_graph_launch", self.handle, g)

    def graph_destroy(self, g):
        self.lib.call("pymes_graph_destroy", self.handle, g)

    def graphs_supported(self):
        return self.lib.backend.startswith("hip")

    def ccsd_energy(self, f, t1, t2):
        e = (C.c_double * 3)()
        self.lib.call("pymes_ccsd_energy", self.handle, C.c_void_p(f.ptr), C.c_void_p(t1.ptr), C.c_void_p(t2.ptr), e)
        return e[0], e[1], e[2]

    def ccd_energy(self, t2):
        e = (C.c_double * 2)()
        self.lib.call("pymes_ccd_energy", self.handle, C.c_void_p(t2.ptr), e)
        return e[0], e[1]

    def dots(self, xs, ys):
        assert len(xs) == len(ys) and all(x.size == y.size for x, y in zip(xs, ys))
        out = np.empty(len(xs))
        for lo in range(0, len(xs), 16):
            hi = min(len(xs), lo + 16)
            buf = (C.c_double * (hi - lo))()
            self.lib.call("pymes_dots_var", self.handle, hi - lo, ptr_array([x.ptr for x in xs[lo:hi]]),
                          ptr_array([y.ptr for y in ys[lo:hi]]), i64_array([x.size for x in xs[lo:hi]]), buf)
            out[lo:hi] = buf[:]
        return out

    def norm(self, x):
        return float(np.sqrt(self.dots([x], [x])[0]))

    def lincomb(self, out, xs, coeffs):
        assert len(xs) == len(coeffs) and all(x.size == out.size for x in xs)
        first = True
        for lo in range(0, len(xs), 7):
            chunk, cc = list(xs[lo:lo + 7]), [float(c) for c in coeffs[lo:lo + 7]]
            if not first:
                chunk, cc = [out] + chunk, [1.0] + cc
            cbuf = (C.c_double * len(cc))(*cc)
            self.lib.call("pymes_lincomb", self.handle, C.c_void_p(out.ptr), len(chunk),
                          ptr_array([x.ptr for x in chunk]), cbuf, out.size)
            first = False
        return out

    def gemm_group(self):
        ctx = self

        class _Group:
            launches = products = 0

            def __enter__(self):
                ctx.lib.call("pymes_gemm_group_begin", ctx.handle)
                return self

            def __exit__(self, *exc):
                l, p = (C.c_int64 * 1)(), (C.c_int64 * 1)()
                ctx.lib.call("pymes_gemm_group_end", ctx.handle, l, p)
                self.launches, self.products = l[0], p[0]
                return False
        return _Group()

    def gram(self, xs, ys):
        m, n = len(xs), len(ys)
        out = np.zeros((m, n))
        if m == 0 or n == 0:
            return out
        size = xs[0].size
        assert all(v.size == size for v in list(xs) + list(ys))
        for i0 in range(0, m, 64):
            for j0 in range(0, n, 64):
                xi, yj = xs[i0:i0 + 64], ys[j0:j0 + 64]
                buf = (C.c_double * (len(xi) * len(yj)))()
                self.lib.call("pymes_gram", self.handle, len(xi), len(yj), ptr_array([x.ptr for x in xi]),
                              ptr_array([y.ptr for y in yj]), size, buf)
                out[i0:i0 + len(xi), j0:j0 + len(yj)] = np.frombuffer(buf, dtype=np.float64).reshape(len(xi), len(yj))
        return out

    def lincomb_multi(self, outs, xs, coeff, beta=None):
        m, n = len(xs), len(outs)
        if n == 0:
            return outs
        coeff = np.ascontiguousarray(np.asarray(coeff, dtype=np.float64).reshape(m, n))
        size = outs[0].size
        assert all(v.size == size for v in list(xs) + list(outs))
        bet = None if beta is None else np.ascontiguousarray(beta, dtype=np.float64)
        for j0 in range(0, n, 64):
            oj = outs[j0:j0 + 64]
            for i0 in range(0, max(m, 1), 64):
                xi = xs[i0:i0 + 64]
                cc = np.ascontiguousarray(coeff[i0:i0 + 64, j0:j0 + 64])
                bb = np.ones(len(oj)) if i0 > 0 else (bet[j0:j0 + 64].copy() if bet is not None else None)
                self.lib.call("pymes_lincomb_multi", self.handle, len(xi), len(oj),
                              ptr_array([x.ptr for x in xi]) if xi else None, _lib.host_ptr(cc) if xi else None,
                              _lib.host_ptr(bb) if bb is not None else None, ptr_array([y.ptr for y in oj]), size)
        return outs

    def diis_mix(self, state_host, err_hist, err_new, amp_hist, outs, m, was_full):
        ntypes = len(err_new)
        assert len(err_hist) == len(amp_hist) == ntypes * m and len(outs) == ntypes and state_host.size >= 96
        self.lib.call("pymes_diis_mix", self.handle, _lib.host_ptr(state_host), ntypes, int(m), int(bool(was_full)),
                      ptr_array([x.ptr for x in err_hist]), ptr_array([x.ptr for x in err_new]),
                      i64_array([x.size for x in err_new]), ptr_array([x.ptr for x in amp_hist]),
                      ptr_array([x.ptr for x in outs]))

    def diis_step(self, state, xs, ys, ntypes, m, was_full):
        assert len(xs) == len(ys) == ntypes * m and state.size >= 96
        self.lib.call("pymes_diis_step", self.handle, C.c_void_p(state.ptr), len(xs), ptr_array([x.ptr for x in xs]),
                      ptr_array([y.ptr for y in ys]), i64_array([x.size for x in xs]), int(ntypes), int(m), int(bool(was_full)))

    def lincomb_dev(self, out, xs, coeff_ptr):
        assert len(xs) <= 8 and all(x.size == out.size for x in xs)
        self.lib.call("pymes_lincomb_dev", self.handle, C.c_void_p(out.ptr), len(xs), ptr_array([x.ptr for x in xs]),
                      C.c_void_p(int(coeff_ptr)), out.size)
        return out

    def cmul(self, mr, mi, xr, xi, yr, yi):
        assert mr.size == mi.size == xr.size == xi.size == yr.size == yi.size
        self.lib.call("pymes_cmul", self.handle, C.c_void_p(mr.ptr), C.c_void_p(mi.ptr), C.c_void_p(xr.ptr), C.c_void_p(xi.ptr),
                      C.c_void_p(yr.ptr), C.c_void_p(yi.ptr), xr.size)

    def cshift_inv(self, d, z, hs, shift, mr, mi):
        z, hs = complex(z), complex(hs)
        self.lib.call("pymes_cshift_inv", self.handle, C.c_void_p(d.ptr), z.real, z.imag, hs.real, hs.imag, float(shift),
                      C.c_void_p(mr.ptr), C.c_void_p(mi.ptr), d.size)

    def stats(self, reset=False):
        gc, pc, gf, pb = C.c_int64(), C.c_int64(), C.c_double(), C.c_double()
        self.lib.call("pymes_stats", self.handle, int(reset), C.byref(gc), C.byref(gf), C.byref(pc), C.byref(pb))
        return {"gemm_calls": gc.value, "gemm_flops": gf.value, "permute_calls": pc.value, "permute_bytes": pb.value}

    def prof_enable(self, on=True):
        self.lib.call("pymes_prof_enable", self.handle, int(on))
# ... 14 lines not shown
```

pymes_amd/mixer/diis.py:

```python
import os

import numpy as np

from pymes_amd import _lib
from pymes_amd.log import print_logging_info

_blas_threads = None


def _single_threaded_blas():
    global _blas_threads
    if _blas_threads is None:
        try:
            from threadpoolctl import ThreadpoolController
            _blas_threads = ThreadpoolController()
        except Exception:
            _blas_threads = False
    if _blas_threads is False:
        import contextlib
        return contextlib.nullcontext()
    return _blas_threads.limit(limits=1, user_api="blas")


class DIIS:
# ... 102 lines not shown
                        vec[k] = ctx.pool_get(arr.shape).set(arr)
                    elif arr.ctx is not ctx:
                        vec[k] = ctx.pool_get(arr.shape).set(arr.get())
        ctx.on_close(self.park)

    def _update_L(self, overlaps, was_full):
        m = len(overlaps)
        L = np.zeros((m + 1, m + 1))
        L[-1, :-1] = -1.0
        L[:-1, -1] = -1.0
        if was_full:
            L[:-3, :-3] = self.L[1:-2, 1:-2]
        else:
            L[:-2, :-2] = self.L[:-1, :-1]
        L[:m, -2] += overlaps
        L[-2, :] = L[:, -2]
        self.L = L.copy()

    def _solve(self):
        with _single_threaded_blas():
            return self._solve_on_this_thread()

    def _solve_on_this_thread(self):
        unit = np.zeros(self.L.shape[0])
        unit[-1] = -1.0
        lam, vec = np.linalg.eigh(self.L)
        if np.any(np.abs(lam) < 1e-12):
            print_logging_info("Linear dependence found in DIIS subspace.", level=2)
            ok = np.abs(lam) > 1e-12
            return np.dot(vec[:, ok] * (1.0 / lam[ok]), np.dot(vec[:, ok].T.conj(), unit))
        return np.linalg.inv(self.L).dot(unit)

    def mix(self, error, amplitude, release=None, sharded=(), allreduce=None, out=None, mark=None, on_device=False,
            defer_log=False, native=False):
        self._adopt(error[0].ctx, error)
        was_full = len(self.error_list) == self.dim_space
        if was_full:
            old_e, old_a = self.error_list.pop(0), self.amplitude_list.pop(0)
            if release is not None:
                for arr in list(old_e) + list(old_a):
                    release(arr)
        self.error_list.append(list(error))
        self.amplitude_list.append(list(amplitude))
        ctx = error[0].ctx
        m, ntypes = len(self.error_list), len(error)
        if on_device and not sharded and ntypes * m <= 16 and m <= 8:
            state = self._device_state(ctx)
            ctx.diis_step(state, [self.error_list[i][nt] for nt in range(ntypes) for i in range(m)],
                          [error[nt] for nt in range(ntypes) for _ in range(m)], ntypes, m, was_full)
            self._stale = True
            self._log_slot = ctx.readback_start(state, 96)
            res = []
            for nt in range(ntypes):
                dst = out[nt] if out is not None else ctx.pool_get(amplitude[nt].shape)
                ctx.lincomb_dev(dst, [self.amplitude_list[a][nt] for a in range(m)], state.ptr + 8 * 82)
                res.append(dst)
            self._log_pending = True
            return res
        self._refresh_host()
        self._state = None
        if native and not sharded and ntypes * m <= 16 and m <= 8:
            buf = np.zeros(96)
            n0 = self.L.shape[0]
            buf[0] = n0
            pad = np.zeros((9, 9))
            pad[:n0, :n0] = self.L
            buf[1:82] = pad.ravel()
            res = [out[nt] if out is not None else ctx.pool_get(amplitude[nt].shape) for nt in range(ntypes)]
            ctx.diis_mix(buf, [self.error_list[i][nt] for nt in range(ntypes) for i in range(m)], list(error),
                         [self.amplitude_list[a][nt] for nt in range(ntypes) for a in range(m)], res, m, was_full)
            n1 = int(buf[0])
            self.L = buf[1:82].reshape(9, 9)[:n1, :n1].copy()
            self.last_coefficients = buf[82:82 + n1].copy()
            self.last_dependent = bool(buf[91] == 1.0)
            if mark is not None:
                mark("DIIS overlaps + host solve (one call)")
            if defer_log:
                self._log_pending = True
            else:
                self.log_last(force=True)
            return res
        overlaps = np.zeros(m)
        parts = ctx.dots([self.error_list[i][nt] for nt in range(ntypes) for i in range(m)],
                         [error[nt] for nt in range(ntypes) for _ in range(m)])
        for nt in range(ntypes):
            part = parts[nt * m:(nt + 1) * m]
            overlaps += allreduce(part) if nt in sharded else part
        if mark is not None:
            mark("DIIS overlaps (reduction + host sync)")
        dependent = False
        if m <= 8 and not os.environ.get("PYMES_NUMPY_DIIS"):
            buf = np.zeros(96)
            n0 = self.L.shape[0]
            buf[0] = n0
            pad = np.zeros((9, 9))
            pad[:n0, :n0] = self.L
            buf[1:82] = pad.ravel()
            ctx.lib.call("pymes_diis_solve", _lib.host_ptr(buf), _lib.host_ptr(np.ascontiguousarray(overlaps, dtype=np.float64)),
                         1, int(m), int(bool(was_full)))
            if buf[91] == 2.0:
                raise np.linalg.LinAlgError("DIIS: the subspace matrix is singular or not finite")
            n1 = int(buf[0])
            self.L = buf[1:82].reshape(9, 9)[:n1, :n1].copy()
            c = buf[82:82 + n1].copy()
            dependent = bool(buf[91] == 1.0)
        else:
            self._update_L(overlaps, was_full)
            c = self._solve()
        self.last_coefficients = c
        if mark is not None:
            mark("DIIS host solve")
        res = []
        for nt in range(ntypes):
            dst = out[nt] if out is not None else ctx.pool_get(amplitude[nt].shape)
            ctx.lincomb(dst, [self.amplitude_list[a][nt] for a in range(m)], c[:m])
            res.append(dst)
        out = res
        if defer_log:
            self._log_pending, self.last_dependent = True, dependent
        else:
            if dependent:
                print_logging_info("Linear dependence found in DIIS subspace.", level=2)
            self._log(c)
        return out

    def _log(self, c):
        print_logging_info("diis.mix", level=2)
        print_logging_info("Coefficients for combining amplitudes=", level=3)
        print_logging_info(c[:-1], level=3)
        print_logging_info("Sum of coefficients = {:.8f}".format(np.sum(c[:-1])), level=3)
        print_logging_info("Lagrangian multiplier = {:.8f}".format(c[-1]), level=3)

    def log_last(self, force=False):
        if getattr(self, "_log_pending", False) or force:
            self._log_pending = False
            self._refresh_host()
            if getattr(self, "last_dependent", False):
                print_logging_info("Linear dependence found in DIIS subspace.", level=2)
            self._log(self.last_coefficients)
```

pymes_amd/solver/ccd.py:

```python
import os
import time

import numpy as np

from pymes_amd.device import Context, DeviceArray, PymesError
from pymes_amd.integral.device import DeviceIntegrals
from pymes_amd.log import print_logging_info
from pymes_amd.mixer import diis


class quiet_collector:

    def __enter__(self):
        import gc
        self.was = gc.isenabled()
        gc.disable()
        return self

    def __exit__(self, *exc):
        if self.was:
            import gc
            gc.enable()
        return False

# ... 106 lines not shown
            print_logging_info("Using DCD: ", self.is_dcd, level=1)
            print_logging_info("Using dr-CCD: ", self.is_dr_ccd, level=1)
            print_logging_info("Solving doubles amplitude equation", level=1)
            print_logging_info("Using data type %s" % ints.dtype, level=1)
            print_logging_info("Using DIIS mixer: ", self.is_diis, level=1)
            print_logging_info("Using Bruekner quasi-particle energy: ", self.is_bruekner, level=1)
            print_logging_info("Iteration = 0", level=1)
            t2 = ctx.pool_get((nv, nv, no, no))
            e_dir, e_exc = ctx.mp2(t2, level_shift)
            e_mp2 = e_dir + e_exc
            print("MP2 energy = ", e_mp2)
            if amps is not None:
                t2.set(np.asarray(amps))
            sym = ctx.V_exchange_symmetric() and (amps is None or ctx.exchange_symmetric(t2))
            dE = np.abs(e_mp2)
            iteration = 0
            e_last = e_mp2
            e_ccd = e_dir_ccd = e_ex_ccd = 0.
            first = True
            shard = self._shard_setup(ctx, t2, sym and amps is None)
            self.pair_sharded = shard is not None
            self.hooked = shard is not None and "coll" in shard
            if shard is None:
                r2 = ctx.pool_get(t2.shape)
                st = {"graph": None, "eager_passes": 0,
                      "graph_ok": ctx.graphs_supported() and not os.environ.get("PYMES_NO_GRAPH")}
                dt_fixed = None if self.is_diis else ctx.pool_get(t2.shape)
            while np.abs(dE) > delta_e and iteration <= max_iter:
                iteration += 1
                if shard is not None:
                    e_dir_ccd, e_ex_ccd, nt, nr = self._sharded_iteration(ctx, shard, f_dev, t2, level_shift, delta)
                else:
                    run_replayable(ctx, st, lambda: ctx.doubles_residual(f_dev, t2, r2, is_dcd=self.is_dcd,
                                                                         sym_ladder=sym))
                    if self.is_diis:
                        t2n, dt2 = ctx.pool_get(t2.shape), ctx.pool_get(t2.shape)
                        ctx.cc_update_to(t2n, dt2, t2, r2, level_shift, delta)
                    else:
                        t2n, dt2 = t2, dt_fixed
                        ctx.cc_update(t2, dt2, r2, level_shift, delta)
                    if first and amps is not None:
                        np.copyto(amps, t2n.get())
                    first = False
                    if self.is_diis:
                        self.mixer.mix([dt2], [t2n], release=ctx.pool_put, out=[t2], defer_log=True,
                                       on_device=bool(os.environ.get("PYMES_DEVICE_DIIS")),
                           native=not os.environ.get("PYMES_NUMPY_DIIS"))
                    _, e_dir_ccd, e_ex_ccd, nt2, nr2, _ = ctx.energy_norms(None, None, t2, dt2)
                    if self.is_diis:
                        self.mixer.log_last()
                    nt, nr = np.sqrt(nt2), np.sqrt(nr2)
                e_ccd = e_dir_ccd + e_ex_ccd
                dE = e_ccd - e_last
                e_last = e_ccd
                if iteration <= max_iter:
                    print_logging_info("Iteration = ", iteration, level=1)
                    print_logging_info("Correlation Energy = {:.12f}".format(e_ccd), level=2)
                    print_logging_info("dE = {:.12e}".format(dE), level=2)
                    print_logging_info("L1 Norm of T2 = {:.12f}".format(nt), level=2)
                    print_logging_info("Norm Residual = {:.12f}".format(nr), level=2)
                else:
                    print_logging_info("A converged solution is not found!", level=1)
            print_logging_info("Direct contribution = {:.12f}".format(e_dir_ccd), level=1)
            print_logging_info("Exchange contribution = {:.12f}".format(e_ex_ccd), level=1)
            print_logging_info("CCD correlation energy = {:.12f}".format(e_ccd), level=1)
            print_logging_info("{:.3f} seconds spent on CCD".format((time.time() - time_ccd)), level=1)
            if amps is not None and not self.is_diis and iteration > 0 and shard is None:
                np.copyto(amps, t2.get())
            result = {"ccd e": e_ccd, "t2 amp": t2.get(), "hole e": t_epsilon_i, "particle e": t_epsilon_a, "dE": dE}
            self.iterations = iteration
            return result
        finally:
            collector.__exit__()
            if own:
                ctx.close()
            elif ctx.handle:
                destroy_graphs(ctx, st)

    def _shard_setup(self, ctx, t2, allowed):
        from pymes_amd import dist as pdist
        from pymes_amd.device import DeviceArray
# ... 127 lines not shown
```

pymes_amd/solver/ccsd.py:

```python
import ctypes as C
import os
import time

import numpy as np

from pymes_amd import _lib
from pymes_amd import dist as pdist
from pymes_amd.device import Context, DeviceArray
from pymes_amd.integral.device import DeviceIntegrals, DressedDeviceIntegrals
from pymes_amd.integral.partition import BLOCK_NAMES
from pymes_amd.log import print_logging_info
from pymes_amd.mixer import diis
from pymes_amd.solver import ccd
from pymes_amd.solver import ccsd_t


DRESSED_KEYS = ("abij", "klij", "ijab", "ijka", "ijak", "iajb", "iabj", "iabc", "abic", "iajk", "abcd")
LOOP_KEYS = ("abij", "klij", "iajb", "iabj", "abcd")


class CCSD(ccd.CCD):
    def __init__(self, no, is_diis=True, delta_e=1.e-8, is_non_canonical=False, is_dcsd=False, device=0,
                 shard_integrals=False):
        self.t_T_ai = None
# ... 69 lines not shown
                st["Xvv_t"], st["Xvv"] = reduced(nv * nv)
                st["P_t"], st["P"] = reduced(ctx.slab_prepare_ws())
                st["R1_t"], st["R1"] = reduced(nv * no)
                st["R1"] = st["R1"].reshape(nv, no)
                if st["pairs"] and not (st["owner_tiles"] and os.environ.get("PYMES_PY_SEQUENCED")):
                    st["S_t"], st["S"] = reduced(8)
                    names = ("ETd", "ETx", "L", "QK", "Tall", "W", "Xvv", "P", "R1", "S")
                    st["coll"] = pdist.Collectives(ctx, {k: st[k + "_t"] for k in names}, rank, wsize)
                    st["bufs"] = _lib.ShardBuffers(*[st[k + "_t"].data_ptr() for k in names])
                    st["rc"] = self._compact(ctx, st)
                    st["flags"] = _lib.PYMES_DCD if self.is_dcd else 0
                    if st["owner_tiles"]:
                        st["coll"].enable_owner_tiles(dev)
                        st["flags"] |= _lib.PYMES_OWNER_TILES
            else:
                st["lad_rows"] = nv * nv
                st["lad_t"], st["lad"] = shared(nv * nv, no * no)
        if not dist_on:
            st["r1"], st["r2"] = ctx.pool_get(t1.shape), ctx.pool_get(t2.shape)
            if not self.is_diis:
                st["dt1"], st["dt2"] = ctx.pool_get(t1.shape), ctx.pool_get(t2.shape)
            st["graph"], st["eager_passes"] = None, 0
            st["eager_passes_of"] = {}
            st["t1_zero"] = amps is None and not os.environ.get("PYMES_NO_T1_SHORTCUT")
            st["graph_ok"] = ctx.graphs_supported() and not os.environ.get("PYMES_NO_GRAPH")
        return st

    def iterate(self, st):
        return self._iterate_sharded(st) if st["dist"] else self._iterate_single(st)

    def _residuals(self, st):
        ctx, t1, t2, r1, r2 = st["ctx"], st["t1"], st["t2"], st["r1"], st["r2"]
        if st["sym"]:
            ctx.ccsd_residuals(st["f"], t1, t2, r1, r2, is_dcd=self.is_dcd, t1_zero=st["t1_zero"])
        else:
            ctx.dress_fock(st["f"], t1, st["fd"])
            ctx.singles_residual(st["fd"], t1, t2, r1)
            ctx.dress_V(t1, LOOP_KEYS)
            ctx.doubles_residual(st["fd"], t2, r2, is_dcd=self.is_dcd, dressed=True, sym_ladder=False)

    def _launch_residuals(self, st):
        ccd.run_replayable(st["ctx"], st, lambda: self._residuals(st), key="t1=0" if st["t1_zero"] else "t1")

    def _iterate_single(self, st):
        ctx, t1, t2, r1, r2 = st["ctx"], st["t1"], st["t2"], st["r1"], st["r2"]
        shift = st["level_shift"]
        mark = pdist.trace.mark
        mark("begin")
        if not st.pop("residuals_in_flight", False):
            self._launch_residuals(st)
        mark("residuals (dressing, R1, R2)")
        with ctx.phase_hold():
            if self.is_diis:
                t1n, t2n, dt1, dt2 = (ctx.pool_get(t1.shape), ctx.pool_get(t2.shape), ctx.pool_get(t1.shape),
                                      ctx.pool_get(t2.shape))
                ctx.cc_update_to(t1n, dt1, t1, r1, shift, self.delta)
                ctx.cc_update_to(t2n, dt2, t2, r2, shift, self.delta)
            else:
                t1n, t2n, dt1, dt2 = t1, t2, st["dt1"], st["dt2"]
                ctx.cc_update(t1, dt1, r1, shift, self.delta)
                ctx.cc_update(t2, dt2, r2, shift, self.delta)
            if st["first"] and st["amps"] is not None:
                np.copyto(st["amps"][0], t1n.get())
                np.copyto(st["amps"][1], t2n.get())
            st["first"] = False
            mark("update")
            if self.is_diis:
                self.mixer.mix([dt1, dt2], [t1n, t2n], release=ctx.pool_put, out=[t1, t2], mark=mark, defer_log=True,
                               on_device=bool(os.environ.get("PYMES_DEVICE_DIIS")),
                               native=not os.environ.get("PYMES_NUMPY_DIIS"))
            mark("DIIS extrapolation")
            slot = ctx.energy_norms_start(st["f"], t1, t2, dt2)
        key = "t1=0" if st["t1_zero"] else "t1"
        speculate = (st.get("speculate", True) and not ctx.profiling and st.get("graphs", {}).get(key) is not None
                     and not os.environ.get("PYMES_NO_PIPELINE"))
        if speculate:
            self._launch_residuals(st)
        e1, ed, ex, nt2, nr2, n1 = ctx.energy_norms_wait(slot)
        mark("energy + norms (read-back) + the next pass's residuals, enqueued ahead" if speculate else "energy + norms (read-back)")
        if self.is_diis:
            self.mixer.log_last()
        was_zero = st["t1_zero"]
        st["t1_zero"] = bool(n1 == 0.0) and not os.environ.get("PYMES_NO_T1_SHORTCUT")
        st["residuals_in_flight"] = bool(speculate and st["t1_zero"] == was_zero)
        return e1, ed, ex, np.sqrt(nt2), np.sqrt(nr2)

    def _hooked_residuals(self, st):
        ctx = st["ctx"]
        st["coll"].call("pymes_ccsd_sharded_residuals", ctx.handle, C.c_void_p(st["f"].ptr), C.c_void_p(st["fd"].ptr),
                        C.c_void_p(st["t1"].ptr), C.c_void_p(st["t2"].ptr), C.byref(st["bufs"]), st["flags"],
                        C.c_void_p(st["rc"].ptr))

    def _iterate_hooked(self, st):
        ctx, t1, tc = st["ctx"], st["t1"], st["Tc"]
        rank, world, shift = st["rank"], st["world"], st["level_shift"]
        coll, mark = st["coll"], pdist.trace.mark
        if not st.pop("residuals_in_flight", False):
            self._hooked_residuals(st)
        dt1, dtc = ctx.pool_get(t1.shape), self._compact(ctx, st)
        ctx.cc_update(t1, dt1, st["R1"], shift, self.delta)
        ctx.cc_update_pairs(tc, dtc, st["rc"], shift, self.delta, rank, world)
        st["first"] = False
        mark("update")
        if self.is_diis:
            t1, tc = self.mixer.mix([dt1, dtc], [t1, tc], release=ctx.pool_put, sharded=(1,),
# ... 480 lines not shown
```

Measured before the change: 0.1616.

## Exploit T2 pair symmetry in update, DIIS, energy/norms and layout kernels

Adds symmetric variants of the T2 amplitude update, DIIS dot products and linear combinations, energy/norm reduction, and pair-layout permutation. They use the t2[a,b,i,j]=t2[b,a,j,i] symmetry to touch roughly half the elements in the memory-bound tail of each CCSD iteration. The new paths are wired through the solver and mixer under a sym_tail switch that can be turned off with an environment variable. The risk is that results are only correct if the amplitudes and residuals really are symmetric.

Result: faster. 0.1594, median of 6 (-1.3%).

```diff
diff --git a/include/pymes_amd.h b/include/pymes_amd.h
--- a/include/pymes_amd.h
+++ b/include/pymes_amd.h
@@ -210,6 +210,19 @@
 int pymes_diis_solve(double* state_host, const double* overlaps_host, int ntypes, int m, int was_full);
 int pymes_lincomb_dev(pymes_ctx* ctx, double* out_dev, int nx, const double* const* x_dev, const double* coeff_dev,
                       int64_t n);
+#define PYMES_SYM_TAIL (1u << 22)
+int pymes_sym_tail(pymes_ctx* ctx, int* yes);
+int pymes_cc_update_to_sym(pymes_ctx* ctx, double* t_out_dev, double* dt_dev, const double* t_in_dev, const double* r_dev,
+                           double level_shift, double delta);
+int pymes_dots_sym(pymes_ctx* ctx, int npairs, const double* const* x_dev, const double* const* y_dev, const int64_t* n,
+                   const int* sym, double* out_host);
+int pymes_lincomb_sym(pymes_ctx* ctx, double* out_dev, int nx, const double* const* x_dev, const double* c_host, int64_t n);
+int pymes_diis_mix_sym(pymes_ctx* ctx, double* state_host, int ntypes, int m, int was_full, const double* const* err_hist_dev,
+                       const double* const* err_new_dev, const int64_t* sizes, const double* const* amp_hist_dev,
+                       double* const* out_dev, const int* sym_types);
+int pymes_energy_norms_start_sym(pymes_ctx* ctx, const double* f_dev, const double* t1_dev, const double* t2_dev,
+                                 const double* dt2_dev, int* slot);
+int pymes_pair_layouts_sym(pymes_ctx* ctx, const double* x_dev, double* Xd_dev, double* Xx_dev, double* Xt_dev);
 int pymes_cmul(pymes_ctx* ctx, const double* mr_dev, const double* mi_dev, const double* xr_dev, const double* xi_dev,
                double* yr_dev, double* yi_dev, int64_t n);
 
diff --git a/pymes_amd/_lib.py b/pymes_amd/_lib.py
--- a/pymes_amd/_lib.py
+++ b/pymes_amd/_lib.py
@@ -181,6 +181,15 @@
     "pymes_gram": (C.c_int, [C.c_void_p, C.c_int, C.c_int, c_pp, c_pp, C.c_int64, c_double_p]),
     "pymes_lincomb_multi": (C.c_int, [C.c_void_p, C.c_int, C.c_int, c_pp, C.c_void_p, C.c_void_p, c_pp, C.c_int64]),
     "pymes_lincomb_dev": (C.c_int, [C.c_void_p, C.c_void_p, C.c_int, c_pp, C.c_void_p, C.c_int64]),
+    "pymes_sym_tail": (C.c_int, [C.c_void_p, C.POINTER(C.c_int)]),
+    "pymes_cc_update_to_sym": (C.c_int, [C.c_void_p, C.c_void_p, C.c_void_p, C.c_void_p, C.c_void_p, C.c_double, C.c_double]),
+    "pymes_dots_sym": (C.c_int, [C.c_void_p, C.c_int, c_pp, c_pp, c_i64_p, C.POINTER(C.c_int), c_double_p]),
+    "pymes_lincomb_sym": (C.c_int, [C.c_void_p, C.c_void_p, C.c_int, c_pp, c_double_p, C.c_int64]),
+    "pymes_diis_mix_sym": (C.c_int, [C.c_void_p, C.c_void_p, C.c_int, C.c_int, C.c_int, c_pp, c_pp, c_i64_p, c_pp, c_pp,
+                                     C.POINTER(C.c_int)]),
+    "pymes_energy_norms_start_sym": (C.c_int, [C.c_void_p, C.c_void_p, C.c_void_p, C.c_void_p, C.c_void_p,
+                                               C.POINTER(C.c_int)]),
+    "pymes_pair_layouts_sym": (C.c_int, [C.c_void_p, C.c_void_p, C.c_void_p, C.c_void_p, C.c_void_p]),
     "pymes_stats": (C.c_int, [C.c_void_p, C.c_int, c_i64_p, c_double_p, c_i64_p, c_double_p]),
     "pymes_prof_enable": (C.c_int, [C.c_void_p, C.c_int]),
     "pymes_prof_reset": (C.c_int, [C.c_void_p]),
@@ -191,6 +200,7 @@
 PYMES_OWNER_TILES = 1 << 21
 PYMES_REUSE_LAYOUTS = 32
 PYMES_T1_ZERO = 1 << 20
+PYMES_SYM_TAIL = 1 << 22
 PYMES_SLAB_RINGS_ONLY, PYMES_SLAB_LADDERS_ONLY = 64, 128
 PYMES_DRESS_ABIJ_REDUCED = 1 << 16
 
diff --git a/pymes_amd/csrc/capi.cpp b/pymes_amd/csrc/capi.cpp
--- a/pymes_amd/csrc/capi.cpp
+++ b/pymes_amd/csrc/capi.cpp
@@ -394,8 +394,10 @@
                          double* r2) {
     return guarded([&] {
         need(f, "f"); need(t1, "t1"); need(t2, "t2"); need(r1, "r1"); need(r2, "r2");
-        if (flags & ~(PYMES_DCD | PYMES_T1_ZERO)) throw pymes::Error("ccsd_residuals: flags are PYMES_DCD | PYMES_T1_ZERO");
-        E(ctx).ccsd_residuals(f, t1, t2, (flags & PYMES_DCD) | ((flags & PYMES_T1_ZERO) ? Engine::kT1Zero : 0u), r1, r2);
+        if (flags & ~(PYMES_DCD | PYMES_T1_ZERO | PYMES_SYM_TAIL))
+            throw pymes::Error("ccsd_residuals: flags are PYMES_DCD | PYMES_T1_ZERO | PYMES_SYM_TAIL");
+        E(ctx).ccsd_residuals(f, t1, t2, (flags & PYMES_DCD) | ((flags & PYMES_T1_ZERO) ? Engine::kT1Zero : 0u) |
+                                             ((flags & PYMES_SYM_TAIL) ? Engine::kSymTail : 0u), r1, r2);
     });
 }
 int pymes_ccsd_iterate(pymes_ctx* ctx, const double* f, double* t1, double* t2, uint32_t flags, double level_shift, double delta,
@@ -649,6 +651,36 @@
         need(t2, "t2"); need(slot, "slot");
         if ((f == nullptr) != (t1 == nullptr)) throw pymes::Error("f and t1 must be given together");
         *slot = E(ctx).energy_norms_start(f, t1, t2, dt2);
+    });
+}
+int pymes_sym_tail(pymes_ctx* ctx, int* yes) {
+    return guarded([&] {
+        need(yes, "yes");
+        *yes = Eq(ctx).sym_tail() ? 1 : 0;
+    });
+}
+int pymes_cc_update_to_sym(pymes_ctx* ctx, double* t_out, double* dt, const double* t_in, const double* r, double shift,
+                           double delta) {
+    return guarded([&] {
+        need(t_out, "t_out"); need(dt, "dt"); need(t_in, "t_in"); need(r, "r");
+        E(ctx).cc_update_to(t_out, dt, t_in, r, shift, delta, 4, true);
+    });
+}
+int pymes_energy_norms_start_sym(pymes_ctx* ctx, const double* f, const double* t1, const double* t2, const double* dt2,
+                                 int* slot) {
+    return guarded([&] {
+        need(t2, "t2"); need(slot, "slot");
+        if ((f == nullptr) != (t1 == nullptr)) throw pymes::Error("f and t1 must be given together");
+        *slot = E(ctx).energy_norms_start(f, t1, t2, dt2, true);
+    });
+}
+int pymes_pair_layouts_sym(pymes_ctx* ctx, const double* x, double* Xd, double* Xx, double* Xt) {
+    return guarded([&] {
+        need(x, "x"); need(Xx, "Xx"); need(Xt, "Xt");
+        Engine& e = E(ctx);
+        if (!dev::fused_pair_kernels_ok(e.no)) throw pymes::Error("pair_layouts: nocc too large for the LDS tile");
+        if (e.sym_tail()) dev::t2_layouts_sym(x, Xd, Xx, Xt, e.no, e.nv, e.stream);
+        else dev::t2_layouts(x, Xd, Xx, Xt, e.no, e.nv, e.stream);
     });
 }
 int pymes_energy_norms_wait(pymes_ctx* ctx, int slot, double* out) {
@@ -852,6 +884,20 @@
         dev::dots(npairs, x, y, n, out, E(ctx).stream);
     });
 }
+int pymes_dots_sym(pymes_ctx* ctx, int npairs, const double* const* x, const double* const* y, const int64_t* n, const int* sym,
+                   double* out) {
+    return guarded([&] {
+        need(x, "x"); need(y, "y"); need(n, "n"); need(sym, "sym"); need(out, "out");
+        if (npairs < 0 || npairs > 16) throw pymes::Error("dots: 0..16 pairs");
+        E(ctx).dots(npairs, x, y, n, sym, out);
+    });
+}
+int pymes_lincomb_sym(pymes_ctx* ctx, double* out, int nx, const double* const* x, const double* c, int64_t n) {
+    return guarded([&] {
+        need(out, "out"); need(x, "x"); need(c, "c");
+        E(ctx).lincomb(out, nx, x, c, n, true);
+    });
+}
 int pymes_lincomb(pymes_ctx* ctx, double* out, int nx, const double* const* x, const double* c, int64_t n) {
     return guarded([&] {
         need(out, "out"); need(x, "x"); need(c, "c");
@@ -907,28 +953,43 @@
         diis_small::step(state_host, overlaps_host, ntypes, m, was_full);
     });
 }
+static void diis_mix_impl(pymes_ctx* ctx, double* state_host, int ntypes, int m, int was_full, const double* const* err_hist,
+                          const double* const* err_new, const int64_t* sizes, const double* const* amp_hist, double* const* out,
+                          const int* sym_types) {
+    need(state_host, "state"); need(err_hist, "err_hist"); need(err_new, "err_new"); need(sizes, "sizes");
+    need(amp_hist, "amp_hist"); need(out, "out");
+    if (ntypes < 1 || m < 1 || m > 8 || ntypes * m > 16) throw pymes::Error("diis_mix: need ntypes * m <= 16, m <= 8");
+    Engine& e = E(ctx);
+    const double* x[16];
+    const double* y[16];
+    int64_t n[16];
+    for (int t = 0; t < ntypes; ++t)
+        for (int i = 0; i < m; ++i) {
+            x[t * m + i] = err_hist[t * m + i];
+            y[t * m + i] = err_new[t];
+            n[t * m + i] = sizes[t];
+        }
+    int sym[16];
+    for (int t = 0; t < ntypes; ++t)
+        for (int i = 0; i < m; ++i) sym[t * m + i] = sym_types ? sym_types[t] : 0;
+    double ov[16];
+    e.dots(ntypes * m, x, y, n, sym, ov);
+    diis_small::step(state_host, ov, ntypes, m, was_full);
+    if (state_host[91] == 2.0)
+        throw pymes::Error("DIIS: the subspace matrix is singular or not finite (numpy.linalg.LinAlgError in pymes/mixer/diis.py:85-95)");
+    for (int t = 0; t < ntypes; ++t)
+        e.lincomb(out[t], m, amp_hist + t * m, state_host + 82, sizes[t], sym_types && sym_types[t]);
+}
 int pymes_diis_mix(pymes_ctx* ctx, double* state_host, int ntypes, int m, int was_full, const double* const* err_hist,
                    const double* const* err_new, const int64_t* sizes, const double* const* amp_hist, double* const* out) {
-    return guarded([&] {
-        need(state_host, "state"); need(err_hist, "err_hist"); need(err_new, "err_new"); need(sizes, "sizes");
-        need(amp_hist, "amp_hist"); need(out, "out");
-        if (ntypes < 1 || m < 1 || m > 8 || ntypes * m > 16) throw pymes::Error("diis_mix: need ntypes * m <= 16, m <= 8");
-        Engine& e = E(ctx);
-        const double* x[16];
-        const double* y[16];
-        int64_t n[16];
-        for (int t = 0; t < ntypes; ++t)
-            for (int i = 0; i < m; ++i) {
-                x[t * m + i] = err_hist[t * m + i];
-                y[t * m + i] = err_new[t];
-                n[t * m + i] = sizes[t];
-            }
-        double ov[16];
-        dev::dots(ntypes * m, x, y, n, ov, e.stream);
-        diis_small::step(state_host, ov, ntypes, m, was_full);
-        if (state_host[91] == 2.0)
-            throw pymes::Error("DIIS: the subspace matrix is singular or not finite (numpy.linalg.LinAlgError in pymes/mixer/diis.py:85-95)");
-        for (int t = 0; t < ntypes; ++t) dev::lincomb(out[t], m, amp_hist + t * m, state_host + 82, sizes[t], e.stream);
+    return guarded([&] { diis_mix_impl(ctx, state_host, ntypes, m, was_full, err_hist, err_new, sizes, amp_hist, out, nullptr); });
+}
+int pymes_diis_mix_sym(pymes_ctx* ctx, double* state_host, int ntypes, int m, int was_full, const double* const* err_hist,
+                       const double* const* err_new, const int64_t* sizes, const double* const* amp_hist, double* const* out,
+                       const int* sym_types) {
+    return guarded([&] {
+        need(sym_types, "sym_types");
+        diis_mix_impl(ctx, state_host, ntypes, m, was_full, err_hist, err_new, sizes, amp_hist, out, sym_types);
     });
 }
 int pymes_lincomb_dev(pymes_ctx* ctx, double* out, int nx, const double* const* x, const double* coeff_dev, int64_t n) {
diff --git a/pymes_amd/csrc/cc.cpp b/pymes_amd/csrc/cc.cpp
--- a/pymes_amd/csrc/cc.cpp
+++ b/pymes_amd/csrc/cc.cpp
@@ -186,7 +186,13 @@
     return true;
 }
 
-void Engine::pair_layouts_of(const double* t2, bool want_td) {
+bool Engine::sym_tail() const {
+    if (const char* e = getenv("PYMES_SYM_TAIL"))
+        if (atoi(e) == 0) return false;
+    return dev::sym_tail_ok() && dev::fused_pair_kernels_ok(no);
+}
+
+void Engine::pair_layouts_of(const double* t2, bool want_td, bool sym) {
     const int64_t o = no, v = nv, ov = o * v;
     for (int i = want_td ? 0 : 1; i < 3; ++i)
         if (!lay_[i]) {
@@ -195,7 +201,8 @@
         }
     lay_t2_ = nullptr;
     if (dev::fused_pair_kernels_ok(no)) {
-        dev::t2_layouts(t2, want_td ? lay_[0] : nullptr, lay_[1], lay_[2], no, nv, stream);
+        if (sym && sym_tail()) dev::t2_layouts_sym(t2, want_td ? lay_[0] : nullptr, lay_[1], lay_[2], no, nv, stream);
+        else dev::t2_layouts(t2, want_td ? lay_[0] : nullptr, lay_[1], lay_[2], no, nv, stream);
         stats.permute_calls++;
         stats.permute_bytes += 8.0 * (want_td ? 5.0 : 4.0) * double(ov * ov);
     } else {
@@ -251,7 +258,7 @@
     auto slab = [&]() { return make_view(arena.alloc(ov * nc), {ov, nc}); };
     const bool traces = !P && nc == ov;
     const bool fold = traces && ring_fold_enabled();
-    pair_layouts_of(t2, !fold);
+    pair_layouts_of(t2, !fold, flags & kSymTail);
     TView Td = pairm(lay_[0]), Tx = pairm(lay_[1]), Ttd = pairm(lay_[2]);
     TView ETd = slice(pairm(ETd_p), 0, c0, c1), ETx = slice(pairm(ETx_p), 0, c0, c1);
     auto cols = [&](const TView& m) { return slice(m, 1, c0, c1); };
@@ -1438,16 +1445,16 @@
         res_fd_ = got[0]; res_ETd_ = got[1]; res_ETx_ = got[2]; res_L_ = got[3]; res_QK_ = got[4];
     }
     const unsigned dcd = flags & PYMES_DCD;
-    const unsigned sym = PYMES_SYM_LADDER | PYMES_SYM_RINGS;
+    const unsigned sym = PYMES_SYM_LADDER | PYMES_SYM_RINGS, tail = flags & kSymTail;
     if (flags & PYMES_T1_ZERO) {
-        residual_slab(f, t2, res_ETd_, res_ETx_, res_L_, 0, 1, dcd | sym);
+        residual_slab(f, t2, res_ETd_, res_ETx_, res_L_, 0, 1, dcd | sym | tail);
         singles_residual_partial(f, t1, t2, r1, 0, 1, true);
         residual_finish(f, t2, res_ETd_, res_ETx_, res_L_, r2, dcd | sym | PYMES_REUSE_LAYOUTS);
         return;
     }
     dress_fock(f, t1, res_fd_);
     dress_V(t1, (1u << pattern_of_name("klij")) | (1u << pattern_of_name("iajb")) | (1u << pattern_of_name("iabj")));
-    residual_slab(res_fd_, t2, res_ETd_, res_ETx_, res_L_, 0, 1, dcd | sym | PYMES_USE_DRESSED, t1, res_QK_);
+    residual_slab(res_fd_, t2, res_ETd_, res_ETx_, res_L_, 0, 1, dcd | sym | tail | PYMES_USE_DRESSED, t1, res_QK_);
     singles_residual_partial(res_fd_, t1, t2, r1, 0, 1, true);
     residual_finish(res_fd_, t2, res_ETd_, res_ETx_, res_L_, r2, dcd | sym | PYMES_USE_DRESSED | PYMES_REUSE_LAYOUTS, t1, res_QK_);
 }
@@ -1467,10 +1474,10 @@
         }
         res_r1_ = r1;
     }
-    ccsd_residuals(f, t1, t2, flags, res_r1_, res_r2_);
+    ccsd_residuals(f, t1, t2, flags | kSymTail, res_r1_, res_r2_);
     cc_update_to(t1, dt1, t1, res_r1_, shift, delta, 2);
-    cc_update_to(t2, dt2, t2, res_r2_, shift, delta, 4);
-    energy_norms(f, t1, t2, dt2, out);
+    cc_update_to(t2, dt2, t2, res_r2_, shift, delta, 4, true);
+    energy_norms(f, t1, t2, dt2, out, true);
 }
 
 void Engine::set_collectives(const Collectives* c) {
@@ -1743,13 +1750,28 @@
 }
 
 void Engine::cc_update_to(double* t_out, double* dt, const double* t_in, const double* r, double shift, double delta,
-                          int rank) {
+                          int rank, bool sym) {
     if (rank != 2 && rank != 4) throw Error("cc_update: rank must be 2 (T1) or 4 (T2)");
     need_eps("cc_update");
-    dev::cc_update_to(t_out, dt, t_in, r, eps_o, eps_v, shift, delta, no, nv, rank, stream);
-}
-
-int Engine::energy_norms_start(const double* f, const double* t1, const double* t2, const double* dt2) {
+    if (sym && rank == 4 && sym_tail()) dev::cc_update_to_sym(t_out, dt, t_in, r, eps_o, eps_v, shift, delta, no, nv, stream);
+    else dev::cc_update_to(t_out, dt, t_in, r, eps_o, eps_v, shift, delta, no, nv, rank, stream);
+}
+
+void Engine::dots(int npairs, const double* const* x, const double* const* y, const int64_t* n, const int* sym, double* out) {
+    bool any = false;
+    for (int i = 0; sym && i < npairs && i < 16; ++i) any = any || sym[i];
+    if (any && sym_tail()) dev::dots_sym(npairs, x, y, n, sym, no, nv, out, stream);
+    else dev::dots(npairs, x, y, n, out, stream);
+}
+
+void Engine::lincomb(double* out, int nx, const double* const* x, const double* c, int64_t n, bool sym) {
+    if (sym && n != (int64_t)nv * nv * no * no) throw Error("lincomb: a symmetric vector must be a [v,v,o,o] array");
+    if (sym && sym_tail()) dev::lincomb_sym(out, nx, x, c, no, nv, stream);
+    else dev::lincomb(out, nx, x, c, n, stream);
+}
+
+int Engine::energy_norms_start(const double* f, const double* t1, const double* t2, const double* dt2, bool sym) {
+    if (sym && sym_tail()) return dev::energy_norms_start_sym(f, t1, t2, get_static("Edir"), get_static("Eex"), dt2, no, nv, stream);
     return dev::energy_norms_start(f, t1, t2, get_static("Edir"), get_static("Eex"), dt2, no, nv, stream);
 }
 void Engine::energy_norms_wait(int slot, double out[6]) {
@@ -1763,7 +1785,8 @@
     out[5] = r[5];
 }
 
-void Engine::energy_norms(const double* f, const double* t1, const double* t2, const double* dt2, double out[6]) {
+void Engine::energy_norms(const double* f, const double* t1, const double* t2, const double* dt2, double out[6], bool sym) {
+    if (sym && sym_tail()) return energy_norms_wait(energy_norms_start(f, t1, t2, dt2, true), out);
     double r[6];
     dev::energy_norms(f, t1, t2, get_static("Edir"), get_static("Eex"), dt2, no, nv, r, stream);
     out[0] = 2.0 * r[0];
diff --git a/pymes_amd/csrc/device_api.h b/pymes_amd/csrc/device_api.h
--- a/pymes_amd/csrc/device_api.h
+++ b/pymes_amd/csrc/device_api.h
@@ -104,6 +104,15 @@
 void cc_update_to(double* t_out, double* dt, const double* t_in, const double* r, const double* eo, const double* ev,
                   double shift, double delta, int no, int nv, int rank, stream_t s);
 void lincomb(double* out, int nx, const double* const* x, const double* c, int64_t n, stream_t s);
+bool sym_tail_ok();
+void cc_update_to_sym(double* t_out, double* dt, const double* t_in, const double* r, const double* eo, const double* ev,
+                      double shift, double delta, int no, int nv, stream_t s);
+void lincomb_sym(double* out, int nx, const double* const* x, const double* c, int no, int nv, stream_t s);
+void dots_sym(int npairs, const double* const* x, const double* const* y, const int64_t* n, const int* sym, int no, int nv,
+              double* out_host, stream_t s);
+int energy_norms_start_sym(const double* f, const double* t1, const double* t2, const double* Edir, const double* Eex,
+                           const double* dt2, int no, int nv, stream_t s);
+void t2_layouts_sym(const double* T, double* Td, double* Tx, double* Ttd, int no, int nv, stream_t s);
 void gram(int m, int n, const double* const* x, const double* const* y, int64_t len, double* out_host, stream_t s);
 void lincomb_multi(int m, int n, const double* const* x, const double* c, const double* beta, double* const* y, int64_t len,
                    stream_t s);
diff --git a/pymes_amd/csrc/engine.cpp b/pymes_amd/csrc/engine.cpp
--- a/pymes_amd/csrc/engine.cpp
+++ b/pymes_amd/csrc/engine.cpp
@@ -787,4 +787,23 @@
 __attribute__((weak)) void tdm1_assemble(const Tdm1Parts&, int, int, int, stream_t) {
     throw std::runtime_error("tdm1_assemble: not available in this backend");
 }
-}
+__attribute__((weak)) bool sym_tail_ok() { return false; }
+__attribute__((weak)) void cc_update_to_sym(double*, double*, const double*, const double*, const double*, const double*, double,
+                                            double, int, int, stream_t) {
+    throw std::runtime_error("cc_update_to_sym: not available in this backend");
+}
+__attribute__((weak)) void lincomb_sym(double*, int, const double* const*, const double*, int, int, stream_t) {
+    throw std::runtime_error("lincomb_sym: not available in this backend");
+}
+__attribute__((weak)) void dots_sym(int, const double* const*, const double* const*, const int64_t*, const int*, int, int, double*,
+                                    stream_t) {
+    throw std::runtime_error("dots_sym: not available in this backend");
+}
+__attribute__((weak)) int energy_norms_start_sym(const double*, const double*, const double*, const double*, const double*,
+                                                 const double*, int, int, stream_t) {
+    throw std::runtime_error("energy_norms_start_sym: not available in this backend");
+}
+__attribute__((weak)) void t2_layouts_sym(const double*, double*, double*, double*, int, int, stream_t) {
+    throw std::runtime_error("t2_layouts_sym: not available in this backend");
+}
+}
diff --git a/pymes_amd/csrc/engine.h b/pymes_amd/csrc/engine.h
--- a/pymes_amd/csrc/engine.h
+++ b/pymes_amd/csrc/engine.h
@@ -162,16 +162,21 @@
                    int64_t q1, bool dcd, const double* J = nullptr);
     void dress_abcd_rows(const double* t1, int a0, int a1, bool lower_only);
     static constexpr unsigned kT1Zero = 1u << 20;
+    static constexpr unsigned kSymTail = 1u << 22;
+    bool sym_tail() const;
     void ccsd_residuals(const double* f, const double* t1, const double* t2, unsigned flags, double* r1, double* r2);
     void ccsd_iterate(const double* f, double* t1, double* t2, unsigned flags, double shift, double delta, double* dt1,
                       double* dt2, double out[6]);
     void release_residual_buffers();
     void cc_update(double* t, double* dt, const double* r, double shift, double delta, int rank);
-    void cc_update_to(double* t_out, double* dt, const double* t_in, const double* r, double shift, double delta, int rank);
+    void cc_update_to(double* t_out, double* dt, const double* t_in, const double* r, double shift, double delta, int rank,
+                      bool sym = false);
+    void dots(int npairs, const double* const* x, const double* const* y, const int64_t* n, const int* sym, double* out);
+    void lincomb(double* out, int nx, const double* const* x, const double* c, int64_t n, bool sym);
     void ccsd_energy(const double* f, const double* t1, const double* t2, double out[3]);
     void ccd_energy(const double* t2, double out[2]);
-    void energy_norms(const double* f, const double* t1, const double* t2, const double* dt2, double out[6]);
-    int energy_norms_start(const double* f, const double* t1, const double* t2, const double* dt2);
+    void energy_norms(const double* f, const double* t1, const double* t2, const double* dt2, double out[6], bool sym = false);
+    int energy_norms_start(const double* f, const double* t1, const double* t2, const double* dt2, bool sym = false);
     void energy_norms_wait(int slot, double out[6]);
     void energy_norms_pairs(const double* f, const double* t1, const double* tc, const double* dtc, int rank, int world,
                             double out[6]);
@@ -217,7 +222,7 @@
   private:
     double* lay_[3] = {nullptr, nullptr, nullptr};
     const double* lay_t2_ = nullptr;
-    void pair_layouts_of(const double* t2, bool want_td);
+    void pair_layouts_of(const double* t2, bool want_td, bool sym = false);
     struct FoldTag {
         const double* t2 = nullptr;
         const double* etd = nullptr;
diff --git a/pymes_amd/csrc/kernels.hip b/pymes_amd/csrc/kernels.hip
--- a/pymes_amd/csrc/kernels.hip
+++ b/pymes_amd/csrc/kernels.hip
@@ -2164,6 +2164,233 @@
     }
 }
 __global__ void __launch_bounds__(256) residual_assemble_kernel(const AssembleK k) { residual_assemble_body(k, blockIdx.x); }
+
+__global__ void __launch_bounds__(256) cc_update_sym_kernel(const CcUpdateK k) {
+    double* t = k.t;
+    double* __restrict__ dt = k.dt;
+    const double* t_in = k.t_in;
+    const double* __restrict__ r_ = k.r;
+    const double* __restrict__ eo = k.eo;
+    const double* __restrict__ ev = k.ev;
+    const double shift = k.shift, delta = k.delta;
+    const int no = k.no, nv = k.nv;
+    extern __shared__ double tile[];
+    int a, b;
+    unrank_pair(blockIdx.x, a, b);
+    const int p = no + 1, o2 = no * no;
+    const long ab = ((long)a * nv + b) * o2, ba = ((long)b * nv + a) * o2;
+    const double eva = ev[a], evb = ev[b];
+    for (int e = threadIdx.x; e < o2; e += blockDim.x) {
+        const int i = e / no, j = e - i * no;
+        const double d = eo[i] + eo[j] - eva - evb;
+        const double inv = 1.0 / (d + shift);
+        const double x = r_[ab + e] * inv;
+        dt[ab + e] = x;
+        tile[i * p + j] = x;
+    }
+    __syncthreads();
+    if (a != b)
+        for (int e = threadIdx.x; e < o2; e += blockDim.x) {
+            const int j = e / no, i = e - j * no;
+            dt[ba + e] = tile[i * p + j];
+        }
+    __syncthreads();
+    for (int e = threadIdx.x; e < o2; e += blockDim.x) {
+        const int i = e / no, j = e - i * no;
+        const double x = tile[i * p + j];
+        const double y = t_in[ab + e] + delta * x;
+        t[ab + e] = y;
+        tile[i * p + j] = y;
+    }
+    __syncthreads();
+    if (a != b)
+        for (int e = threadIdx.x; e < o2; e += blockDim.x) {
+            const int j = e / no, i = e - j * no;
+            t[ba + e] = tile[i * p + j];
+        }
+}
+
+struct LinSymK {
+    double* out;
+    LinPtrs p;
+    int nx, no, nv;
+};
+__global__ void __launch_bounds__(256) lincomb_sym_kernel(const LinSymK k) {
+    double* out = k.out;
+    const int nx = k.nx, no = k.no, nv = k.nv;
+    extern __shared__ double tile[];
+    int a, b;
+    unrank_pair(blockIdx.x, a, b);
+    const int p = no + 1, o2 = no * no;
+    const long ab = ((long)a * nv + b) * o2, ba = ((long)b * nv + a) * o2;
+    for (int e = threadIdx.x; e < o2; e += blockDim.x) {
+        const int i = e / no, j = e - i * no;
+        double s = 0.0;
+        for (int q = 0; q < nx; ++q) s += k.p.x[q][ab + e] * k.p.c[q];
+        out[ab + e] = s;
+        tile[i * p + j] = s;
+    }
+    if (a == b) return;
+    __syncthreads();
+    for (int e = threadIdx.x; e < o2; e += blockDim.x) {
+        const int j = e / no, i = e - j * no;
+        out[ba + e] = tile[i * p + j];
+    }
+}
+
+__global__ void __launch_bounds__(256) t2_layouts_sym_kernel(const LayoutsK k) {
+    const double* __restrict__ T = k.T;
+    double* __restrict__ Td = k.Td;
+    double* __restrict__ Tx = k.Tx;
+    double* __restrict__ Ttd = k.Ttd;
+    const int no = k.no, nv = k.nv;
+    extern __shared__ double tile[];
+    const int a = blockIdx.x / nv, b = blockIdx.x - a * nv;
+    const int p = no + 1, o2 = no * no;
+    const long ov = (long)no * nv;
+    const double* __restrict__ Tab = T + ((long)a * nv + b) * o2;
+    const long base = (long)a * no * ov + (long)b * no;
+    for (int e = threadIdx.x; e < o2; e += blockDim.x) {
+        const int i = e / no, j = e - i * no;
+        const double x = Tab[e];
+        tile[i * p + j] = x;
+        if (Td) Td[base + (long)i * ov + j] = x;
+    }
+    __syncthreads();
+    for (int e = threadIdx.x; e < o2; e += blockDim.x) {
+        const int i = e / no, j = e - i * no;
+        Ttd[base + (long)i * ov + j] = 2.0 * tile[i * p + j] - tile[j * p + i];
+    }
+    for (int e = threadIdx.x; e < o2; e += blockDim.x) {
+        const int j = e / no, i = e - j * no;
+        Tx[base + (long)j * ov + i] = tile[i * p + j];
+    }
+}
+
+struct DotsSymK {
+    DotsK d;
+    unsigned symmask;
+    int o2, nv;
+};
+template <int VEC, int SVEC>
+__global__ void __launch_bounds__(256) dots_stage1_sym_kernel(const DotsSymK k) {
+    __shared__ double sh[4];
+    const int nb = k.d.nb, npairs = k.d.npairs;
+    const int lin = blockIdx.x;
+    int pair, b;
+    if ((nb & 7) == 0) { const int q = lin >> 3; pair = q % npairs; b = (q / npairs) * 8 + (lin & 7); }
+    else { pair = lin / nb; b = lin - pair * nb; }
+    if (!((k.symmask >> pair) & 1u)) {
+        dots_stage1_body<VEC>(k.d, blockIdx.x, sh);
+        return;
+    }
+    const double* __restrict__ x = k.d.p.x[pair];
+    const double* __restrict__ y = k.d.p.y[pair];
+    const int o2 = k.o2, nv = k.nv;
+    const long npp = (long)nv * (nv + 1) / 2;
+    double off = 0.0, dia = 0.0;
+    for (long t = b; t < npp; t += nb) {
+        int va, vb;
+        unrank_pair(t, va, vb);
+        const long base = ((long)va * nv + vb) * o2;
+        double s = 0.0;
+        if (SVEC == 2) {
+            const double2* __restrict__ x2 = reinterpret_cast<const double2*>(x + base);
+            const double2* __restrict__ y2 = reinterpret_cast<const double2*>(y + base);
+            double s1 = 0.0;
+#pragma unroll 4
+            for (int i = threadIdx.x; i < (o2 >> 1); i += 256) {
+                const double2 u = x2[i], w = y2[i];
+                s += u.x * w.x;
+                s1 += u.y * w.y;
+            }
+            s += s1;
+        } else {
+#pragma unroll 4
+            for (int i = threadIdx.x; i < o2; i += 256) s += x[base + i] * y[base + i];
+        }
+        if (va == vb) dia += s;
+        else off += s;
+    }
+    const double r_off = block_sum(off, sh), r_dia = block_sum(dia, sh);
+    if (threadIdx.x == 0) k.d.partial[pair * kDotBlocks + b] = 2.0 * r_off + r_dia;
+}
+
+template <int VEC>
+__global__ void __launch_bounds__(256) energy_norms_sym_kernel(const EnergyK k) {
+    __shared__ double sh[4];
+    const double* __restrict__ f = k.f;
+    const double* __restrict__ t1 = k.t1;
+    const double* __restrict__ t2 = k.t2;
+    const double* __restrict__ Edir = k.Edir;
+    const double* __restrict__ Eex = k.Eex;
+    const double* __restrict__ dt2 = k.dt2;
+    double* __restrict__ partial = k.partial;
+    const int no = k.no, nv = k.nv;
+    const unsigned vb = blockIdx.x, vgrid = gridDim.x;
+    const int noV = no / VEC, o2V = no * noV;
+    const int sj = 256 % noV, si = 256 / noV;
+    const long npp = (long)nv * (nv + 1) / 2;
+    double s0 = 0.0, s5 = 0.0;
+    double o1 = 0.0, o2 = 0.0, o3 = 0.0, o4 = 0.0, d1 = 0.0, d2 = 0.0, d3 = 0.0, d4 = 0.0;
+    for (long t = vb; t < npp; t += vgrid) {
+        int a, b;
+        unrank_pair(t, a, b);
+        const long base = ((long)a * nv + b) * no * no;
+        double s1 = 0.0, s2 = 0.0, s3 = 0.0, s4 = 0.0;
+        int i = (int)threadIdx.x / noV, j = (int)threadIdx.x - i * noV;
+#pragma unroll 2
+        for (int e = threadIdx.x; e < o2V; e += 256) {
+            if (VEC == 2) {
+                const double2 x = reinterpret_cast<const double2*>(t2 + base)[e];
+                const double2 ed = reinterpret_cast<const double2*>(Edir + base)[e], ex = reinterpret_cast<const double2*>(Eex + base)[e];
+                double tx = x.x, ty = x.y;
+                if (t1) {
+                    const double ta = t1[a * no + i];
+                    tx += ta * t1[b * no + 2 * j];
+                    ty += ta * t1[b * no + 2 * j + 1];
+                }
+                s1 += tx * ed.x + ty * ed.y;
+                s2 += tx * ex.x + ty * ex.y;
+                s3 += x.x * x.x + x.y * x.y;
+                if (dt2) { const double2 d = reinterpret_cast<const double2*>(dt2 + base)[e]; s4 += d.x * d.x + d.y * d.y; }
+            } else {
+                const double x = t2[base + e];
+                double tau = x;
+                if (t1) tau += t1[a * no + i] * t1[b * no + j];
+                s1 += tau * Edir[base + e];
+                s2 += tau * Eex[base + e];
+                s3 += x * x;
+                if (dt2) { const double d = dt2[base + e]; s4 += d * d; }
+            }
+            j += sj;
+            const int c = j >= noV; j -= c ? noV : 0;
+            i += si + c;
+        }
+        if (a == b) { d1 += s1; d2 += s2; d3 += s3; d4 += s4; }
+        else { o1 += s1; o2 += s2; o3 += s3; o4 += s4; }
+    }
+    if (t1 && f) {
+        const long n = no + nv, ov = (long)no * nv;
+        for (long e = vb * (long)blockDim.x + threadIdx.x; e < ov; e += (long)vgrid * blockDim.x) {
+            const long a = e / no, i = e - a * no;
+            const double y = t1[e];
+            s0 += f[i * n + no + a] * y;
+            s5 += y * y;
+        }
+    }
+    const double r0 = block_sum(s0, sh), r5 = block_sum(s5, sh);
+    const double r1 = 2.0 * block_sum(o1, sh) + block_sum(d1, sh), r2 = 2.0 * block_sum(o2, sh) + block_sum(d2, sh),
+                 r3 = 2.0 * block_sum(o3, sh) + block_sum(d3, sh), r4 = 2.0 * block_sum(o4, sh) + block_sum(d4, sh);
+    if (threadIdx.x == 0) {
+        partial[5 * kDotBlocks + vb] = r5;
+        partial[0 * kDotBlocks + vb] = r0;
+        partial[1 * kDotBlocks + vb] = r1;
+        partial[2 * kDotBlocks + vb] = r2;
+        partial[3 * kDotBlocks + vb] = r3;
+        partial[4 * kDotBlocks + vb] = r4;
+    }
+}
 
 __global__ void __launch_bounds__(256) energy_norms_pairs_kernel(const double* __restrict__ f, const double* __restrict__ t1,
                                                                  const double* __restrict__ tc, const double* __restrict__ Edir,
@@ -4263,9 +4490,23 @@
                double delta, int no, int nv, int rank, stream_t s) {
     cc_update_to(t, dt, t, r, eo, ev, shift, delta, no, nv, rank, s);
 }
+void cc_update_to_sym(double* t_out, double* dt, const double* t_in, const double* r, const double* eo, const double* ev,
+                      double shift, double delta, int no, int nv, stream_t s) {
+    if (!fused_pair_kernels_ok(no)) throw std::runtime_error("cc_update_to_sym: nocc too large for the LDS tile");
+    const long total = (long)nv * nv * no * no;
+    if (!total) return;
+    phase_open((hipStream_t)s);
+    if (phase_small(32.0 * (double)total / 4.0e6)) {
+        cc_update_to(t_out, dt, t_in, r, eo, ev, shift, delta, no, nv, 4, s);
+        return;
+    }
+    const CcUpdateK k{t_out, dt, t_in, r, eo, ev, shift, delta, no, nv, 4, total};
+    launch_kernel(cc_update_sym_kernel, dim3((unsigned)((long)nv * (nv + 1) / 2)), dim3(256), sizeof(double) * no * (no + 1),
+                  (hipStream_t)s, k);
+}
 
 static int launch_dots_stage1(int npairs, const double* const* x, const double* const* y, const int64_t* n, double* ws,
-                              hipStream_t st) {
+                              hipStream_t st, unsigned symmask = 0u, int no = 0, int nv = 0) {
     DotPtrs p;
     long nmax = 0;
     bool vec = true;
@@ -4292,6 +4533,13 @@
         phase_writes(t, {prange(ws, 16L * kDotBlocks)});
         return nb;
     }
+    if (symmask && !phase_small(bytes / 4.0e6)) {
+        const DotsSymK ks{k, symmask, no * no, nv};
+        if (vec && even((long)no * no)) launch_kernel(dots_stage1_sym_kernel<2, 2>, dim3(nb * npairs), dim3(256), 0, st, ks);
+        else if (vec) launch_kernel(dots_stage1_sym_kernel<2, 1>, dim3(nb * npairs), dim3(256), 0, st, ks);
+        else launch_kernel(dots_stage1_sym_kernel<1, 1>, dim3(nb * npairs), dim3(256), 0, st, ks);
+        return nb;
+    }
     if (vec) launch_kernel(dots_stage1_kernel<2>, dim3(nb * npairs), dim3(256), 0, st, k);
     else launch_kernel(dots_stage1_kernel<1>, dim3(nb * npairs), dim3(256), 0, st, k);
     return nb;
@@ -4321,13 +4569,14 @@
     launch_kernel(dots_final_kernel, dim3(k.npairs), dim3(256), 0, st, k);
 }
 
-void dots(int npairs, const double* const* x, const double* const* y, const int64_t* n, double* out_host, stream_t s) {
+static void dots_impl(int npairs, const double* const* x, const double* const* y, const int64_t* n, unsigned symmask, int no,
+                      int nv, double* out_host, stream_t s) {
     if (npairs <= 0) return;
     if (npairs > 16) throw std::runtime_error("dots: at most 16 pairs per call");
     hipStream_t st = (hipStream_t)s;
     const int dv = current_device();
     ensure_dot_ws(dv);
-    const int nb = launch_dots_stage1(npairs, x, y, n, g_dot_ws[dv], st);
+    const int nb = launch_dots_stage1(npairs, x, y, n, g_dot_ws[dv], st, symmask, no, nv);
     void* hd = nullptr;
     HIP_CHECK(hipHostGetDevicePointer(&hd, g_dot_host[dv], 0));
     const long seq = ++g_dot_seq[dv];
@@ -4337,6 +4586,20 @@
     phase_flush();
     if (!poll_flag(reinterpret_cast<const long*>(g_dot_host[dv] + 16), seq, st)) throw std::runtime_error("dots: the device never delivered the result");
     for (int i = 0; i < npairs; ++i) out_host[i] = g_dot_host[dv][i];
+}
+void dots(int npairs, const double* const* x, const double* const* y, const int64_t* n, double* out_host, stream_t s) {
+    dots_impl(npairs, x, y, n, 0u, 0, 0, out_host, s);
+}
+bool sym_tail_ok() { return true; }
+void dots_sym(int npairs, const double* const* x, const double* const* y, const int64_t* n, const int* sym, int no, int nv,
+              double* out_host, stream_t s) {
+    unsigned mask = 0u;
+    for (int i = 0; i < npairs && i < 16; ++i)
+        if (sym[i]) {
+            if (n[i] != (int64_t)nv * nv * no * no) throw std::runtime_error("dots_sym: a symmetric pair is not [nv,nv,no,no]");
+            mask |= 1u << i;
+        }
+    dots_impl(npairs, x, y, n, mask, no, nv, out_host, s);
 }
 
 void diis_step(double* state, int npairs, const double* const* x, const double* const* y, const int64_t* n, int ntypes, int m,
@@ -4360,8 +4623,8 @@
     launch_kernel(lincomb_dev_kernel, dim3(grid_for(n)), dim3(256), 0, (hipStream_t)s, out, p, coeff_dev, nx, (long)n);
 }
 
-int energy_norms_start(const double* f, const double* t1, const double* t2, const double* Edir, const double* Eex,
-                       const double* dt2, int no, int nv, stream_t s) {
+static int energy_norms_start_impl(const double* f, const double* t1, const double* t2, const double* Edir, const double* Eex,
+                                   const double* dt2, int no, int nv, bool sym, stream_t s) {
     gemm_group_flush();
     hipStream_t st = (hipStream_t)s;
     const int dv = current_device();
@@ -4378,6 +4641,9 @@
         phase_reads(t, {prange(t2, total), prange(Edir, total), prange(Eex, total), prange(dt2, dt2 ? total : 0),
                         prange(t1, t1 ? (long)no * nv : 0), prange(f, (t1 && f) ? n * n : 0)});
         phase_writes(t, {prange(g_dot_ws[dv], 16L * kDotBlocks)});
+    } else if (sym && total && !phase_small(cost)) {
+        if (vec) launch_kernel(energy_norms_sym_kernel<2>, dim3(nb), dim3(256), 0, st, k);
+        else launch_kernel(energy_norms_sym_kernel<1>, dim3(nb), dim3(256), 0, st, k);
     } else {
         if (vec) launch_kernel(energy_norms_kernel<2>, dim3(nb), dim3(256), 0, st, k);
         else launch_kernel(energy_norms_kernel<1>, dim3(nb), dim3(256), 0, st, k);
@@ -4389,6 +4655,14 @@
     launch_dots_final(DotsFinalK{g_dot_ws[dv], out_pin, flag, nullptr, 0u, seq, nb, 6}, g_dot_ws[dv], st);
     phase_flush();
     return ticket;
+}
+int energy_norms_start(const double* f, const double* t1, const double* t2, const double* Edir, const double* Eex,
+                       const double* dt2, int no, int nv, stream_t s) {
+    return energy_norms_start_impl(f, t1, t2, Edir, Eex, dt2, no, nv, false, s);
+}
+int energy_norms_start_sym(const double* f, const double* t1, const double* t2, const double* Edir, const double* Eex,
+                           const double* dt2, int no, int nv, stream_t s) {
+    return energy_norms_start_impl(f, t1, t2, Edir, Eex, dt2, no, nv, true, s);
 }
 void energy_norms(const double* f, const double* t1, const double* t2, const double* Edir, const double* Eex,
                   const double* dt2, int no, int nv, double out_host[6], stream_t s) {
@@ -4439,6 +4713,22 @@
         return;
     }
     launch_kernel(lincomb_kernel, dim3(grid_for(n)), dim3(256), 0, (hipStream_t)s, k);
+}
+void lincomb_sym(double* out, int nx, const double* const* x, const double* c, int no, int nv, stream_t s) {
+    if (nx < 0 || nx > 8) throw std::runtime_error("lincomb: at most 8 terms");
+    if (!fused_pair_kernels_ok(no)) throw std::runtime_error("lincomb_sym: nocc too large for the LDS tile");
+    const long n = (long)nv * nv * no * no;
+    if (n <= 0) return;
+    phase_open((hipStream_t)s);
+    if (phase_small(8.0 * (double)(nx + 1) * (double)n / 4.0e6)) {
+        lincomb(out, nx, x, c, n, s);
+        return;
+    }
+    LinPtrs p;
+    for (int i = 0; i < 8; ++i) { p.x[i] = i < nx ? x[i] : nullptr; p.c[i] = i < nx ? c[i] : 0.0; }
+    const LinSymK k{out, p, nx, no, nv};
+    launch_kernel(lincomb_sym_kernel, dim3((unsigned)((long)nv * (nv + 1) / 2)), dim3(256), sizeof(double) * no * (no + 1),
+                  (hipStream_t)s, k);
 }
 
 namespace {
@@ -4755,6 +5045,18 @@
     }
     if (res) launch_kernel(t2_layouts_kernel<true>, dim3((unsigned)(nv * nv)), dim3(256), lds, (hipStream_t)s, k);
     else launch_kernel(t2_layouts_kernel<false>, dim3((unsigned)(nv * nv)), dim3(256), lds, (hipStream_t)s, k);
+}
+void t2_layouts_sym(const double* T, double* Td, double* Tx, double* Ttd, int no, int nv, stream_t s) {
+    if (!fused_pair_kernels_ok(no)) throw std::runtime_error("t2_layouts: nocc too large for the LDS tile");
+    const long n4 = (long)nv * nv * no * no;
+    phase_open((hipStream_t)s);
+    if (phase_small(40.0 * (double)n4 / 4.0e6)) {
+        t2_layouts(T, Td, Tx, Ttd, no, nv, s);
+        return;
+    }
+    if (!n4) return;
+    const LayoutsK k{T, Td, Tx, Ttd, 2.0, -1.0, no, nv};
+    launch_kernel(t2_layouts_sym_kernel, dim3((unsigned)(nv * nv)), dim3(256), sizeof(double) * no * (no + 1), (hipStream_t)s, k);
 }
 
 void residual_assemble(const double* V, const double* L, const double* N, const double* D, const double* X, double* R,
diff --git a/pymes_amd/device.py b/pymes_amd/device.py
--- a/pymes_amd/device.py
+++ b/pymes_amd/device.py
@@ -361,10 +361,15 @@
         else:
             self.lib.call("pymes_ccsd_dress_V", self.handle, C.c_void_p(t1.ptr), mask)
 
-    def ccsd_residuals(self, f, t1, t2, r1, r2, is_dcd=False, t1_zero=False):
+    def ccsd_residuals(self, f, t1, t2, r1, r2, is_dcd=False, t1_zero=False, sym_tail=False):
         self.lib.call("pymes_ccsd_residuals", self.handle, C.c_void_p(f.ptr), C.c_void_p(t1.ptr), C.c_void_p(t2.ptr),
-                      (_lib.PYMES_DCD if is_dcd else 0) | (_lib.PYMES_T1_ZERO if t1_zero else 0), C.c_void_p(r1.ptr),
-                      C.c_void_p(r2.ptr))
+                      (_lib.PYMES_DCD if is_dcd else 0) | (_lib.PYMES_T1_ZERO if t1_zero else 0) |
+                      (_lib.PYMES_SYM_TAIL if sym_tail else 0), C.c_void_p(r1.ptr), C.c_void_p(r2.ptr))
+
+    def sym_tail(self):
+        yes = C.c_int()
+        self.lib.call("pymes_sym_tail", self.handle, C.byref(yes))
+        return bool(yes.value)
 
     def ccsd_iterate(self, f, t1, t2, dt1, dt2, level_shift=0.0, delta=1.0, is_dcd=False, t1_zero=False):
         out = (C.c_double * 6)()
@@ -388,11 +393,11 @@
         return out
 
     def doubles_residual(self, f, t2, out, is_dcd=False, dressed=False, skip_ladder=False, sym_ladder=False,
-                         sym_rings=None):
+                         sym_rings=None, sym_tail=False):
         sym_rings = sym_ladder if sym_rings is None else sym_rings
         flags = (_lib.PYMES_DCD if is_dcd else 0) | (_lib.PYMES_USE_DRESSED if dressed else 0) | \
                 (_lib.PYMES_SKIP_LADDER if skip_ladder else 0) | (_lib.PYMES_SYM_LADDER if sym_ladder else 0) | \
-                (_lib.PYMES_SYM_RINGS if sym_rings else 0)
+                (_lib.PYMES_SYM_RINGS if sym_rings else 0) | (_lib.PYMES_SYM_TAIL if sym_tail and sym_rings else 0)
         self.lib.call("pymes_doubles_residual", self.handle, C.c_void_p(f.ptr), C.c_void_p(t2.ptr),
                       C.c_void_p(out.ptr), flags)
         return out
@@ -498,8 +503,8 @@
                       C.c_void_p(W.ptr), int(ld), int(r0), int(r1), int(minus_half))
         return W
 
-    def pair_layouts(self, x, Xx, Xt, Xd=None):
-        self.lib.call("pymes_pair_layouts", self.handle, C.c_void_p(x.ptr), C.c_void_p(Xd.ptr if Xd is not None else 0),
+    def pair_layouts(self, x, Xx, Xt, Xd=None, sym=False):
+        self.lib.call("pymes_pair_layouts_sym" if sym else "pymes_pair_layouts", self.handle, C.c_void_p(x.ptr), C.c_void_p(Xd.ptr if Xd is not None else 0),
                       C.c_void_p(Xx.ptr), C.c_void_p(Xt.ptr))
 
     def symmetrised_assemble(self, N, D, X, out, V=None, L=None):
@@ -524,25 +529,33 @@
         self.lib.call("pymes_ladder_sym_unpack", self.handle, C.c_void_p(L.ptr), C.c_void_p(out.ptr), float(beta))
         return out
 
-    def cc_update(self, t, dt, r, level_shift=0.0, delta=1.0):
+    def cc_update(self, t, dt, r, level_shift=0.0, delta=1.0, sym=False):
         rank = len(t.shape)
+        if sym and rank == 4:
+            return self.cc_update_to(t, dt, t, r, level_shift, delta, sym=True)
         self.lib.call("pymes_cc_update", self.handle, C.c_void_p(t.ptr), C.c_void_p(dt.ptr), C.c_void_p(r.ptr),
                       float(level_shift), float(delta), rank)
 
-    def cc_update_to(self, t_out, dt, t_in, r, level_shift=0.0, delta=1.0):
+    def cc_update_to(self, t_out, dt, t_in, r, level_shift=0.0, delta=1.0, sym=False):
+        if sym and len(t_in.shape) == 4:
+            self.lib.call("pymes_cc_update_to_sym", self.handle, C.c_void_p(t_out.ptr), C.c_void_p(dt.ptr),
+                          C.c_void_p(t_in.ptr), C.c_void_p(r.ptr), float(level_shift), float(delta))
+            return
         self.lib.call("pymes_cc_update_to", self.handle, C.c_void_p(t_out.ptr), C.c_void_p(dt.ptr), C.c_void_p(t_in.ptr),
                       C.c_void_p(r.ptr), float(level_shift), float(delta), len(t_in.shape))
 
-    def energy_norms(self, f, t1, t2, dt2=None):
+    def energy_norms(self, f, t1, t2, dt2=None, sym=False):
+        if sym:
+            return self.energy_norms_wait(self.energy_norms_start(f, t1, t2, dt2, sym=True))
         out = (C.c_double * 6)()
         self.lib.call("pymes_energy_norms", self.handle, C.c_void_p(f.ptr if f is not None else 0),
                       C.c_void_p(t1.ptr if t1 is not None else 0), C.c_void_p(t2.ptr),
                       C.c_void_p(dt2.ptr if dt2 is not None else 0), out)
         return tuple(out[:])
 
-    def energy_norms_start(self, f, t1, t2, dt2=None):
+    def energy_norms_start(self, f, t1, t2, dt2=None, sym=False):
         slot = C.c_int()
-        self.lib.call("pymes_energy_norms_start", self.handle, C.c_void_p(f.ptr if f is not None else 0),
+        self.lib.call("pymes_energy_norms_start_sym" if sym else "pymes_energy_norms_start", self.handle, C.c_void_p(f.ptr if f is not None else 0),
                       C.c_void_p(t1.ptr if t1 is not None else 0), C.c_void_p(t2.ptr),
                       C.c_void_p(dt2.ptr if dt2 is not None else 0), C.byref(slot))
         return slot.value
@@ -605,12 +618,18 @@
         self.lib.call("pymes_ccd_energy", self.handle, C.c_void_p(t2.ptr), e)
         return e[0], e[1]
 
-    def dots(self, xs, ys):
+    def dots(self, xs, ys, sym=None):
         assert len(xs) == len(ys) and all(x.size == y.size for x, y in zip(xs, ys))
         out = np.empty(len(xs))
         for lo in range(0, len(xs), 16):
             hi = min(len(xs), lo + 16)
             buf = (C.c_double * (hi - lo))()
+            if sym is not None and any(sym[lo:hi]):
+                self.lib.call("pymes_dots_sym", self.handle, hi - lo, ptr_array([x.ptr for x in xs[lo:hi]]),
+                              ptr_array([y.ptr for y in ys[lo:hi]]), i64_array([x.size for x in xs[lo:hi]]),
+                              (C.c_int * (hi - lo))(*[int(bool(f)) for f in sym[lo:hi]]), buf)
+                out[lo:hi] = buf[:]
+                continue
             self.lib.call("pymes_dots_var", self.handle, hi - lo, ptr_array([x.ptr for x in xs[lo:hi]]),
                           ptr_array([y.ptr for y in ys[lo:hi]]), i64_array([x.size for x in xs[lo:hi]]), buf)
             out[lo:hi] = buf[:]
@@ -619,7 +638,7 @@
     def norm(self, x):
         return float(np.sqrt(self.dots([x], [x])[0]))
 
-    def lincomb(self, out, xs, coeffs):
+    def lincomb(self, out, xs, coeffs, sym=False):
         assert len(xs) == len(coeffs) and all(x.size == out.size for x in xs)
         first = True
         for lo in range(0, len(xs), 7):
@@ -627,7 +646,7 @@
             if not first:
                 chunk, cc = [out] + chunk, [1.0] + cc
             cbuf = (C.c_double * len(cc))(*cc)
-            self.lib.call("pymes_lincomb", self.handle, C.c_void_p(out.ptr), len(chunk),
+            self.lib.call("pymes_lincomb_sym" if sym else "pymes_lincomb", self.handle, C.c_void_p(out.ptr), len(chunk),
                           ptr_array([x.ptr for x in chunk]), cbuf, out.size)
             first = False
         return out
@@ -684,9 +703,16 @@
                               _lib.host_ptr(bb) if bb is not None else None, ptr_array([y.ptr for y in oj]), size)
         return outs
 
-    def diis_mix(self, state_host, err_hist, err_new, amp_hist, outs, m, was_full):
+    def diis_mix(self, state_host, err_hist, err_new, amp_hist, outs, m, was_full, sym_types=None):
         ntypes = len(err_new)
         assert len(err_hist) == len(amp_hist) == ntypes * m and len(outs) == ntypes and state_host.size >= 96
+        if sym_types is not None and any(sym_types):
+            assert len(sym_types) == ntypes
+            self.lib.call("pymes_diis_mix_sym", self.handle, _lib.host_ptr(state_host), ntypes, int(m), int(bool(was_full)),
+                          ptr_array([x.ptr for x in err_hist]), ptr_array([x.ptr for x in err_new]),
+                          i64_array([x.size for x in err_new]), ptr_array([x.ptr for x in amp_hist]),
+                          ptr_array([x.ptr for x in outs]), (C.c_int * ntypes)(*[int(bool(f)) for f in sym_types]))
+            return
         self.lib.call("pymes_diis_mix", self.handle, _lib.host_ptr(state_host), ntypes, int(m), int(bool(was_full)),
                       ptr_array([x.ptr for x in err_hist]), ptr_array([x.ptr for x in err_new]),
                       i64_array([x.size for x in err_new]), ptr_array([x.ptr for x in amp_hist]),
diff --git a/pymes_amd/mixer/diis.py b/pymes_amd/mixer/diis.py
--- a/pymes_amd/mixer/diis.py
+++ b/pymes_amd/mixer/diis.py
@@ -158,7 +158,7 @@
         return np.linalg.inv(self.L).dot(unit)
 
     def mix(self, error, amplitude, release=None, sharded=(), allreduce=None, out=None, mark=None, on_device=False,
-            defer_log=False, native=False):
+            defer_log=False, native=False, sym=()):
         self._adopt(error[0].ctx, error)
         was_full = len(self.error_list) == self.dim_space
         if was_full:
@@ -194,7 +194,8 @@
             buf[1:82] = pad.ravel()
             res = [out[nt] if out is not None else ctx.pool_get(amplitude[nt].shape) for nt in range(ntypes)]
             ctx.diis_mix(buf, [self.error_list[i][nt] for nt in range(ntypes) for i in range(m)], list(error),
-                         [self.amplitude_list[a][nt] for nt in range(ntypes) for a in range(m)], res, m, was_full)
+                         [self.amplitude_list[a][nt] for nt in range(ntypes) for a in range(m)], res, m, was_full,
+                         sym_types=[nt in sym for nt in range(ntypes)] if sym and not sharded else None)
             n1 = int(buf[0])
             self.L = buf[1:82].reshape(9, 9)[:n1, :n1].copy()
             self.last_coefficients = buf[82:82 + n1].copy()
@@ -208,7 +209,8 @@
             return res
         overlaps = np.zeros(m)
         parts = ctx.dots([self.error_list[i][nt] for nt in range(ntypes) for i in range(m)],
-                         [error[nt] for nt in range(ntypes) for _ in range(m)])
+                         [error[nt] for nt in range(ntypes) for _ in range(m)],
+                         sym=[nt in sym for nt in range(ntypes) for _ in range(m)] if sym and not sharded else None)
         for nt in range(ntypes):
             part = parts[nt * m:(nt + 1) * m]
             overlaps += allreduce(part) if nt in sharded else part
@@ -239,7 +241,7 @@
         res = []
         for nt in range(ntypes):
             dst = out[nt] if out is not None else ctx.pool_get(amplitude[nt].shape)
-            ctx.lincomb(dst, [self.amplitude_list[a][nt] for a in range(m)], c[:m])
+            ctx.lincomb(dst, [self.amplitude_list[a][nt] for a in range(m)], c[:m], sym=bool(nt in sym and not sharded))
             res.append(dst)
         out = res
         if defer_log:
diff --git a/pymes_amd/solver/ccd.py b/pymes_amd/solver/ccd.py
--- a/pymes_amd/solver/ccd.py
+++ b/pymes_amd/solver/ccd.py
@@ -162,21 +162,21 @@
                     e_dir_ccd, e_ex_ccd, nt, nr = self._sharded_iteration(ctx, shard, f_dev, t2, level_shift, delta)
                 else:
                     run_replayable(ctx, st, lambda: ctx.doubles_residual(f_dev, t2, r2, is_dcd=self.is_dcd,
-                                                                         sym_ladder=sym))
+                                                                         sym_ladder=sym, sym_tail=sym))
                     if self.is_diis:
                         t2n, dt2 = ctx.pool_get(t2.shape), ctx.pool_get(t2.shape)
-                        ctx.cc_update_to(t2n, dt2, t2, r2, level_shift, delta)
+                        ctx.cc_update_to(t2n, dt2, t2, r2, level_shift, delta, sym=sym)
                     else:
                         t2n, dt2 = t2, dt_fixed
-                        ctx.cc_update(t2, dt2, r2, level_shift, delta)
+                        ctx.cc_update(t2, dt2, r2, level_shift, delta, sym=sym)
                     if first and amps is not None:
                         np.copyto(amps, t2n.get())
                     first = False
                     if self.is_diis:
                         self.mixer.mix([dt2], [t2n], release=ctx.pool_put, out=[t2], defer_log=True,
                                        on_device=bool(os.environ.get("PYMES_DEVICE_DIIS")),
-                           native=not os.environ.get("PYMES_NUMPY_DIIS"))
-                    _, e_dir_ccd, e_ex_ccd, nt2, nr2, _ = ctx.energy_norms(None, None, t2, dt2)
+                           native=not os.environ.get("PYMES_NUMPY_DIIS"), sym=(0,) if sym else ())
+                    _, e_dir_ccd, e_ex_ccd, nt2, nr2, _ = ctx.energy_norms(None, None, t2, dt2, sym=sym)
                     if self.is_diis:
                         self.mixer.log_last()
                     nt, nr = np.sqrt(nt2), np.sqrt(nr2)
diff --git a/pymes_amd/solver/ccsd.py b/pymes_amd/solver/ccsd.py
--- a/pymes_amd/solver/ccsd.py
+++ b/pymes_amd/solver/ccsd.py
@@ -125,7 +125,7 @@
     def _residuals(self, st):
         ctx, t1, t2, r1, r2 = st["ctx"], st["t1"], st["t2"], st["r1"], st["r2"]
         if st["sym"]:
-            ctx.ccsd_residuals(st["f"], t1, t2, r1, r2, is_dcd=self.is_dcd, t1_zero=st["t1_zero"])
+            ctx.ccsd_residuals(st["f"], t1, t2, r1, r2, is_dcd=self.is_dcd, t1_zero=st["t1_zero"], sym_tail=True)
         else:
             ctx.dress_fock(st["f"], t1, st["fd"])
             ctx.singles_residual(st["fd"], t1, t2, r1)
@@ -138,6 +138,7 @@
     def _iterate_single(self, st):
         ctx, t1, t2, r1, r2 = st["ctx"], st["t1"], st["t2"], st["r1"], st["r2"]
         shift = st["level_shift"]
+        sym = bool(st["sym"])
         mark = pdist.trace.mark
         mark("begin")
         if not st.pop("residuals_in_flight", False):
@@ -148,11 +149,11 @@
                 t1n, t2n, dt1, dt2 = (ctx.pool_get(t1.shape), ctx.pool_get(t2.shape), ctx.pool_get(t1.shape),
                                       ctx.pool_get(t2.shape))
                 ctx.cc_update_to(t1n, dt1, t1, r1, shift, self.delta)
-                ctx.cc_update_to(t2n, dt2, t2, r2, shift, self.delta)
+                ctx.cc_update_to(t2n, dt2, t2, r2, shift, self.delta, sym=sym)
             else:
                 t1n, t2n, dt1, dt2 = t1, t2, st["dt1"], st["dt2"]
                 ctx.cc_update(t1, dt1, r1, shift, self.delta)
-                ctx.cc_update(t2, dt2, r2, shift, self.delta)
+                ctx.cc_update(t2, dt2, r2, shift, self.delta, sym=sym)
             if st["first"] and st["amps"] is not None:
                 np.copyto(st["amps"][0], t1n.get())
                 np.copyto(st["amps"][1], t2n.get())
@@ -161,9 +162,9 @@
             if self.is_diis:
                 self.mixer.mix([dt1, dt2], [t1n, t2n], release=ctx.pool_put, out=[t1, t2], mark=mark, defer_log=True,
                                on_device=bool(os.environ.get("PYMES_DEVICE_DIIS")),
-                               native=not os.environ.get("PYMES_NUMPY_DIIS"))
+                               native=not os.environ.get("PYMES_NUMPY_DIIS"), sym=(1,) if sym else ())
             mark("DIIS extrapolation")
-            slot = ctx.energy_norms_start(st["f"], t1, t2, dt2)
+            slot = ctx.energy_norms_start(st["f"], t1, t2, dt2, sym=sym)
         key = "t1=0" if st["t1_zero"] else "t1"
         speculate = (st.get("speculate", True) and not ctx.profiling and st.get("graphs", {}).get(key) is not None
                      and not os.environ.get("PYMES_NO_PIPELINE"))
```
